# zhiyuns/AFCM

Measured on AMD Instinct MI355X. Metric: generator fwd+bwd images/sec @256^2, higher is better.
Workload: dtype bf16; 1 GPU; AFCM --model stylegan3 generator training step (fwd + L1 loss + bwd + grad all-reduce + Adam), IXI T1->T2 shape: 256x256, 4->1 channels, full-width 58.5M-param generator, random init; global_batch=16, per_gpu_batch=16, resolution=256, parallelism=dp1, world_size=1, gradient_buckets=0, comm_dtype=fp32, homogeneous_dot=True

## Files before the change

### afcm_amd/_lib.py

```python
import ctypes as C
import os

import torch

_HERE = os.path.dirname(os.path.abspath(__file__))
LIB_PATH = os.environ.get('AFCM_HIP_LIB') or os.path.join(_HERE, 'libafcm_hip.so')

F32, F16, BF16 = 0, 1, 2
E_NOKERNEL, E_INVALID = -1, -2
SIGNS_NONE, SIGNS_WRITE, SIGNS_READ = 0, 1, 2

_DTYPES = {torch.float32: F32, torch.float16: F16, torch.bfloat16: BF16}


class FilteredLReluArgs(C.Structure):
    _fields_ = [
        ('x', C.c_void_p), ('y', C.c_void_p), ('b', C.c_void_p), ('signs', C.c_void_p),
        ('fu', C.c_void_p), ('fd', C.c_void_p),
        ('dtype', C.c_int32),
        ('n', C.c_int32), ('c', C.c_int32), ('xh', C.c_int32), ('xw', C.c_int32), ('yh', C.c_int32), ('yw', C.c_int32),
        ('fuw', C.c_int32), ('fuh', C.c_int32), ('fdw', C.c_int32), ('fdh', C.c_int32),
        ('up', C.c_int32), ('down', C.c_int32),
        ('px0', C.c_int32), ('px1', C.c_int32), ('py0', C.c_int32), ('py1', C.c_int32),
        ('sx', C.c_int32), ('sy', C.c_int32), ('sh', C.c_int32), ('swb', C.c_int32),
        ('gain', C.c_float), ('slope', C.c_float), ('clamp', C.c_float),
        ('flip_filter', C.c_int32), ('sign_mode', C.c_int32),
        ('workspace', C.c_void_p), ('sign_layout', C.c_int32), ('plane_sum_slots', C.c_int32),
        ('plane_sum', C.c_void_p), ('oscale', C.c_void_p), ('skip', C.c_void_p), ('oscale2', C.c_void_p),
        ('x_pitch', C.c_int32), ('y_pitch', C.c_int32), ('skip_pitch', C.c_int32), ('row_pitch_ok', C.c_int32),
        ('clamp_flags', C.c_void_p),
    ]


AFFINE_MAX = 16


class AffineBank(C.Structure):
    _fields_ = [
        ('layers', C.c_int32), ('n', C.c_int32), ('kw', C.c_int32), ('kg', C.c_int32),
        ('w_stride_n', C.c_int64), ('w_stride_l', C.c_int64),
        ('w', C.c_void_p), ('g', C.c_void_p),
        ('weight', C.c_void_p * AFFINE_MAX), ('bias', C.c_void_p * AFFINE_MAX),
        ('cout', C.c_int32 * AFFINE_MAX), ('w_index', C.c_int32 * AFFINE_MAX),
        ('alpha', C.c_float * AFFINE_MAX), ('beta', C.c_float * AFFINE_MAX),
    ]


MODULATION_MAX = 16


class ModulationLayer(C.Structure):
    _fields_ = [('cout', C.c_int32), ('cin', C.c_int32), ('kk', C.c_int32), ('demodulate', C.c_int32)] + [
        (k, C.c_void_p) for k in ('w', 't', 'magnitude', 'w_hat', 'wsq', 'scale', 's_eff', 'd', 'r', 'g_hat', 'g_s', 'g_d', 'dw', 'dt', 'workspace')]


PACK_MAX = 32


class PackEntry(C.Structure):
    _fields_ = [('dst_fwd', C.c_void_p), ('dst_dgrad', C.c_void_p), ('w', C.c_void_p),
                ('cout', C.c_int32), ('cin', C.c_int32), ('rows_pad_fwd', C.c_int32), ('rows_pad_dgrad', C.c_int32)]


_lib = None
ABI_VERSION = 13

_i32, _i64, _f32, _vp = C.c_int32, C.c_int64, C.c_float, C.c_void_p
SIGNATURES = {
    'afcm_abi_version': (C.c_int, []),
    'afcm_last_error': (C.c_char_p, []),
    'afcm_noop': (C.c_int, [_vp]),
    'afcm_filtered_lrelu_shapes': (C.c_int, [C.POINTER(FilteredLReluArgs)]),
    'afcm_filtered_lrelu': (C.c_int, [C.POINTER(FilteredLReluArgs), _vp]),
    'afcm_filtered_lrelu_workspace_bytes': (C.c_int64, []),
    'afcm_filtered_lrelu_prepare': (C.c_int, [C.POINTER(FilteredLReluArgs), _vp]),
    'afcm_filtered_lrelu_act': (C.c_int, [_vp, _vp, _i32, _i32, _i32, _i32, _i32, _i32, _i32, _i32, _i32, _f32, _f32, _f32, _i32, _vp]),
    'afcm_upfirdn2d': (C.c_int, [_vp, _vp, _vp, _i32, _i32, _i32, _i32, _i32, _i32, _i32, _i32, _i32, _i32, _i32, _i32, _i32,
                                 _i32, _i32, _i32, _f32, _vp]),
    'afcm_bias_act': (C.c_int, [_vp, _vp, _vp, _vp, _vp, _vp, _i32, _i64, _i64, _i32, _i32, _i32, _f32, _f32, _f32, _vp]),
    'afcm_conv2d_block_k': (C.c_int, [_i32]),
    'afcm_conv2d_block_k_ks': (C.c_int, [_i32, _i32]),
    'afcm_conv2d_pack_weights_bk': (C.c_int, [_vp, _vp, _i32, _i32, _i32, _i32, _i32, _i32, _i32, _vp]),
    'afcm_conv2d_pack_weights': (C.c_int, [_vp, _vp, _i32, _i32, _i32, _i32, _i32, _i32, _vp]),
    'afcm_conv2d_pack_weights2': (C.c_int, [_vp, _vp, _vp, _i32, _i32, _i32, _i32, _i32, _i32, _vp]),
    'afcm_conv2d': (C.c_int, [_vp, _vp, _vp, _vp, _vp, _i32, _i32, _i32, _i32, _i32, _i32, _i32, _i32, _i32, _vp]),
    'afcm_conv2d_ld': (C.c_int, [_vp, _vp, _vp, _vp, _vp, _i32, _i32, _i32, _i32, _i32, _i32, _i32, _i32, _i32, _i32, _i32, _vp]),
    'afcm_conv2d_wgrad_splits': (C.c_int, [_i32, _i32, _i32, _i32]),
    'afcm_conv2d_wgrad': (C.c_int, [_vp, _vp, _vp, _vp, _i32, _i32, _i32, _i32, _i32, _i32, _i32, _i32, _vp]),
    'afcm_conv2d_wgrad_ld': (C.c_int, [_vp, _vp, _vp, _vp, _i32, _i32, _i32, _i32, _i32, _i32, _i32, _i32, _i32, _i32, _vp]),
    'afcm_conv2d_wgrad_dots_ld': (C.c_int, [_vp, _vp, _vp, _vp, _vp, _vp, _i32, _i32, _i32, _i32, _i32, _i32, _i32, _i32, _i32, _i32, _vp]),
    'afcm_scale_planes': (C.c_int, [_vp, _vp, _vp, _i32, _i32, _i64, _i32, _vp]),
    'afcm_plane_dot': (C.c_int, [_vp, _vp, _vp, _i32, _i64, _i32, _vp]),
    'afcm_plane_dot_ld': (C.c_int, [_vp, _vp, _vp, _i32, _i64, _i32, _i32, _i32, _i32, _vp]),
    'afcm_split16': (C.c_int, [_vp, _vp, _vp, _vp, _i32, _i64, _i32, _i32, _i64, _vp]),
    'afcm_conv2d_split': (C.c_int, [_vp, _vp, _vp, _vp, _vp, _i32, _i32, _i32, _i32, _i32, _i32, _i32, _i32, _i32, C.c_uint32, _i64, _vp, _vp, _vp]),
    'afcm_amax_bits': (C.c_int, [_vp, _vp, _i64, _i32, _vp, _vp]),
    'afcm_unscale': (C.c_int, [_vp, _i64, _vp, _vp, _vp]),
    'afcm_plane_dot_parts': (C.c_int, [_vp, _vp, _i64, _i32, _vp, _i32, _i64, _i32, _vp, _vp]),
    'afcm_conv2d_pack_split': (C.c_int, [_vp, _vp, _vp, _i32, _i32, _i32, _i32, _i32, _i32, C.c_uint32, _vp]),
    'afcm_plane_dot_gated_ld': (C.c_int, [_vp, _vp, _vp, _i32, _i64, _i32, _i32, _i32, _i32, _vp, _i32, _vp, _vp, _vp, _vp, _vp]),
    'afcm_weight_norm_fwd': (C.c_int, [_vp, _vp, _vp, _vp, _i32, _i32, _i32, _vp]),
    'afcm_weight_norm_bwd': (C.c_int, [_vp, _vp, _vp, _vp, _vp, _i32, _i32, _i32, _vp]),
    'afcm_style_coefs_fwd': (C.c_int, [_vp, _vp, _vp, _vp, _vp, _vp, _i32, _i32, _i32, _i32, _vp]),
    'afcm_style_coefs_bwd': (C.c_int, [_vp, _vp, _vp, _vp, _vp, _vp, _vp, _vp, _vp, _vp, _i32, _i32, _i32, _i32, _vp]),
    'afcm_layer_bwd_coefs': (C.c_int, [_vp, _vp, _vp, _vp, _i32, _vp, _vp, _vp, _vp, _vp, _i32, _i32, _vp]),
    'afcm_affine_bank_workspace_bytes': (C.c_int64, [C.POINTER(AffineBank)]),
    'afcm_affine_bank_fwd': (C.c_int, [C.POINTER(AffineBank), C.POINTER(C.c_void_p), _vp]),
    'afcm_modulation_bank_workspace_floats': (C.c_int64, [_i32, _i32, _i32, _i32]),
    'afcm_modulation_bank_fwd': (C.c_int, [C.POINTER(ModulationLayer), _i32, _i32, _vp]),
    'afcm_modulation_bank_bwd': (C.c_int, [C.POINTER(ModulationLayer), _i32, _i32, _vp]),
    'afcm_conv2d_stride2': (C.c_int, [_vp, _vp, _vp, _i32, _i32, _i32, _i32, _i32, _i32, _i32, _i32, _vp]),
    'afcm_conv2d_pack_bank': (C.c_int, [C.POINTER(PackEntry), _i32, _i32, _i32, _vp]),
    'afcm_affine_bank_bwd': (C.c_int, [C.POINTER(AffineBank), C.POINTER(C.c_void_p), C.POINTER(C.c_void_p), C.POINTER(C.c_void_p), _vp, _vp, _vp, _vp]),
    'afcm_pool_blocks_fwd': (C.c_int, [_vp, _vp, _i32, _i64, _i32, _i32, _vp]),
    'afcm_pool_blocks_bwd': (C.c_int, [_vp, _vp, _i32, _i64, _i32, _i32, _vp]),
    'afcm_l1_partials': (C.c_int, [_vp, _vp, _vp, _i64, _i32, _f32, _vp]),
    'afcm_l1_grad': (C.c_int, [_vp, _vp, _vp, _vp, _i64, _f32, _vp]),
    'afcm_axpy_planes': (C.c_int, [_vp, _vp, _vp, _vp, _i32, _i64, _i32, _vp]),
    'afcm_fc_act_fwd': (C.c_int, [_vp, _vp, _vp, _vp, _i32, _i32, _i32, _f32, _f32, _i32, _vp]),
    'afcm_fc_act_bwd': (C.c_int, [_vp, _vp, _vp, _vp, _vp, _vp, _vp, _i32, _i32, _i32, _f32, _f32, _i32, _vp]),
    'afcm_mapping_input_fwd': (C.c_int, [_vp, _vp, _vp, _vp, _vp, _i32, _i32, _i32, _i32, _f32, _f32, _vp]),
    'afcm_mapping_input_bwd_workspace_bytes': (C.c_int64, [_i32, _i32]),
    'afcm_mapping_input_bwd': (C.c_int, [_vp, _vp, _vp, _vp, _vp, _vp, _i32, _i32, _i32, _i32, _f32, _f32, _vp, _vp]),
    'afcm_adam_chunk_elems': (C.c_int32, []),
    'afcm_adam_multi': (C.c_int, [_vp, _i32, _i64, _f32, _f32, _f32, _f32, _f32, _f32, _f32, _f32, _i32, _f32, _f32, _i32, _vp]),
    'afcm_adam_multi_capturable': (C.c_int, [_vp, _i32, _i64, _vp, _f32, _f32, _f32, _f32, _f32, _i32, _f32, _f32, _i32, _vp]),
}


def load():
    global _lib
    if _lib is None:
        if not os.path.exists(LIB_PATH):
            raise RuntimeError(
                f'{LIB_PATH} is missing: the HIP kernels are not built.  Run `python -c "import __graft_entry__ as g; g.build()"` '
                f'or `make -C afcm_amd/csrc`.  afcm_amd has no CPU fallback.')
        lib = C.CDLL(LIB_PATH)
        for name, (res, args) in SIGNATURES.items():
            fn = getattr(lib, name)
            fn.restype = res
            fn.argtypes = args
        if lib.afcm_abi_version() != ABI_VERSION:
            raise RuntimeError(f'libafcm_hip.so ABI version {lib.afcm_abi_version()} does not match this package ({ABI_VERSION}); rebuild it')
        _lib = lib
    return _lib


def dtype_code(t):
    try:
        return _DTYPES[t.dtype]
    except KeyError:
        raise RuntimeError(f'afcm_amd kernels support float32/float16/bfloat16, got {t.dtype}') from None


def require_gpu(*tensors):
    for t in tensors:
        if t is not None and t.device.type != 'cuda':
            raise RuntimeError(
                f'afcm_amd ops need ROCm device tensors (got a tensor on {t.device}); there is no CPU path in this package '
                f'-- the aten reference lives in oracle/ and is test-only')


def stream_ptr(t):
    return torch.cuda.current_stream(t.device).cuda_stream


def ptr(t):
    return None if t is None else t.data_ptr()


def check(rc, what):
    if rc == 0 or rc == E_NOKERNEL:
        return rc
    if rc == E_INVALID:
        raise RuntimeError(f'{what}: {load().afcm_last_error().decode()}')
    raise RuntimeError(f'{what}: HIP error {rc - 1000} at kernel launch')


def launched(rc, what):
    if check(rc, what) == E_NOKERNEL:
        raise RuntimeError(f'{what}: no kernel for this shape (the Python gate and the C entry point disagree)')
    return rc
```

### afcm_amd/csrc/conv2d.hip

```cpp
#include <stdlib.h>
#include <string.h>

#include <type_traits>

#include "common.h"

namespace afcm {

typedef __attribute__((ext_vector_type(16))) float f32x16;
typedef __attribute__((ext_vector_type(8))) __bf16 bf16x8;
typedef __attribute__((ext_vector_type(8))) _Float16 f16x8;
typedef __attribute__((ext_vector_type(2))) float cf32x2;
typedef __attribute__((ext_vector_type(2))) __bf16 cbf16x2;
typedef __attribute__((ext_vector_type(2))) _Float16 cf16x2;

template <typename T>
__device__ __forceinline__ unsigned pack2(float lo, float hi) {
    if constexpr (std::is_same<T, bf16_t>::value) {
        union { cbf16x2 v; unsigned u; } r;
        r.v = __builtin_convertvector((cf32x2){lo, hi}, cbf16x2);
        return r.u;
    } else {
        union { cf16x2 v; unsigned u; } r;
        r.v = __builtin_convertvector((cf32x2){lo, hi}, cf16x2);
        return r.u;
    }
}

template <typename T> struct ConvCfg;
template <> struct ConvCfg<bf16_t> { static constexpr int BK = 16, PITCH = 24; };
template <> struct ConvCfg<f16_t>  { static constexpr int BK = 16, PITCH = 24; };
template <> struct ConvCfg<float>  { static constexpr int BK = 8,  PITCH = 9;  };

static inline int conv_bk(int dtype, int ks);
int conv2d_direct_small_cin(const void* x, void* y, const void* wp, const float* oscale, const float* obias, int dtype, int n, int cin, int cout,
                            int h, int w, int pad, int rows_pad, int bk, int ldx, int ldy, hipStream_t st);

constexpr int kPatchMax = 416;
constexpr int kPlaneX16 = 416;
constexpr int kPatchMaxX16 = kPlaneX16 - 4;
constexpr int kPatchMaxS2 = 704;
constexpr int kSlots = 256;

struct ConvParams {
    const void* x;
    void* y;
    const void* wp;
    const float* oscale;
    const float* obias;
    int N, Cin, Cout, H, W, P, Q;
    int ldx, ldy;
    int pad;
    int TH, TW, PWL, tilesX, tilesY;
    int Opad, nkc;
    int total_blocks;
    int o_base;
    unsigned magicTW;
    unsigned magicTX, magicTY, magicN, magicPC;
    int nkc_real; unsigned magicNK, term_parts; int part_bytes, last_part_bytes;
    const unsigned* bound_a; const unsigned* bound_b;
};
__device__ __forceinline__ float pow2_factor(unsigned bound_bits, float* inverse = nullptr) {
    const float b = __uint_as_float(bound_bits);
    int e = 15;
    if (b <= 3.4028234664e38f) frexpf(fmaxf(b, 1e-30f), &e);
    if (inverse) *inverse = ldexpf(1.f, e - 15);
    return ldexpf(1.f, 15 - e);
}

__host__ __device__ inline unsigned magic_u32(unsigned d) { return (unsigned)((0x100000000ull + d - 1) / d); }
__device__ __forceinline__ unsigned udiv_magic(unsigned n, unsigned magic) { return magic ? __umulhi(n, magic) : n; }

template <typename T, int BM_O, int KS>
__global__ __launch_bounds__(256, (sizeof(T) == 4 ? 1 : 2)) void conv2d_fwd_kernel(ConvParams p) {
    typedef ConvCfg<T> C;
    constexpr int BK = C::BK, PITCH = C::PITCH, MI = BM_O / 64, KK = KS * KS;
    constexpr bool F32 = sizeof(T) == 4;
    constexpr int EPV = 16 / sizeof(T);
    constexpr int PPR = BK / EPV;
    constexpr int NPIECES = KK * BM_O * PPR;
    constexpr int NWP = cdiv(NPIECES, 256);
    __shared__ __attribute__((aligned(16))) T lds[(KK * BM_O + kPatchMax) * PITCH];
    T* lds_w = lds;
    T* lds_p = lds + KK * BM_O * PITCH;

    const int tid = threadIdx.x, lane = tid & 63, wave = tid >> 6;
    const int wo = wave & 1, wpx = wave >> 1;
    const int r32 = lane & 31, h = lane >> 5;

    int bid = blockIdx.x;
    const int tx = __builtin_amdgcn_readfirstlane(bid % p.tilesX); bid /= p.tilesX;
    const int ty = __builtin_amdgcn_readfirstlane(bid % p.tilesY); bid /= p.tilesY;
    const int n = __builtin_amdgcn_readfirstlane(bid % p.N);
    const int ob = __builtin_amdgcn_readfirstlane(bid / p.N);
    const int y0 = ty * p.TH, x0 = tx * p.TW;
    const int o0 = ob * BM_O;
    const int PH = p.TH + KS - 1, PWL = p.PWL;
    const int xorg = (x0 - p.pad) & ~1;
    const int xoff = (x0 - p.pad) - xorg;

    int bbase[4], pyv[4], pxv[4];
#pragma unroll
    for (int ti = 0; ti < 4; ti++) {
        const int j = wpx * 128 + ti * 32 + r32;
        int py = j / p.TW, px = j - py * p.TW;
        const bool valid = j < p.TH * p.TW;
        if (!valid) { py = 0; px = 0; }
        pyv[ti] = valid ? y0 + py : p.P;
        pxv[ti] = x0 + px;
        bbase[ti] = (py * PWL + px + xoff) * PITCH + h * (F32 ? 1 : 8);
    }
    int abase[MI];
#pragma unroll
    for (int mi = 0; mi < MI; mi++) abase[mi] = (wo * (BM_O / 2) + mi * 32 + r32) * PITCH + h * (F32 ? 1 : 8);

    f32x16 acc[MI][4];
#pragma unroll
    for (int mi = 0; mi < MI; mi++)
#pragma unroll
        for (int ti = 0; ti < 4; ti++)
#pragma unroll
            for (int e = 0; e < 16; e++) acc[mi][ti][e] = 0.f;

    constexpr int PPT = BM_O * PPR;
    constexpr int TPI = 256 / PPT;
    const int wq = tid % PPT, wtap0 = tid / PPT;
    const int wsrc0 = ((wtap0 * p.Opad) + o0 + wq / PPR) * BK + (wq % PPR) * EPV;
    const int wdst0 = (wtap0 * BM_O + wq / PPR) * PITCH + (wq % PPR) * EPV;
    const int wsrc_step = TPI * p.Opad * BK, wdst_step = TPI * BM_O * PITCH;
    const size_t wchunk = (size_t)KK * p.Opad * BK;
    const int cg = F32 ? 0 : (tid >> 5) & 1, pg = F32 ? tid : (tid & 31) + 32 * (tid >> 6);
    const int pcols = PWL >> 2;
    const int prow = pg / pcols, pcol4 = pg - prow * pcols;
    const bool pvalid = prow < PH;
    const int iy = y0 - p.pad + prow, ix = xorg + 4 * pcol4;
    const bool rowok = pvalid && (unsigned)iy < (unsigned)p.H;
    const T* xn = (const T*)p.x + (size_t)n * p.Cin * p.H * p.W;
    const long long pix_off = (long long)(rowok ? iy : 0) * p.W + ix;
    const int pdst = (prow * PWL + 4 * pcol4) * PITCH + cg * 8;

    unsigned wreg[NWP][4];
    unsigned preg[8][F32 ? 4 : 2];
    constexpr unsigned kOob = 0x80000000u;
    const bool d0ok = rowok && (unsigned)ix < (unsigned)p.W, d1ok = rowok && (unsigned)(ix + 2) < (unsigned)p.W;
    const unsigned pmask0 = d0ok ? ~0u : 0u, pmask1 = d1ok ? ~0u : 0u;
    const bool any_partial = __builtin_amdgcn_ballot_w64(d0ok != d1ok) != 0;
    const bool lshift = !d0ok && d1ok;
    const bool any_lshift = __builtin_amdgcn_ballot_w64(lshift) != 0;
    const unsigned pvoff = (d0ok || d1ok) ? (unsigned)(((long long)cg * 8 * p.H * p.W + pix_off + (lshift ? 2 : 0)) * (long long)sizeof(T)) : kOob;
    const long long img_bytes = (long long)p.Cin * p.H * p.W * (long long)sizeof(T);
    const __amdgpu_buffer_rsrc_t xrs = __builtin_amdgcn_make_buffer_rsrc((void*)xn, 0, (int)(img_bytes > 0x7fffffffll ? 0x7fffffffll : img_bytes), 0x00020000);
    const int hw2 = p.H * p.W * (int)sizeof(T);

    auto issue_loads = [&](int kc) __attribute__((always_inline)) {
        const T* wsrcp = (const T*)p.wp + (size_t)kc * wchunk;
#pragma unroll
        for (int i = 0; i < NWP; i++)
            if ((NPIECES % 256 == 0) || tid + i * 256 < NPIECES) {
                const uint4 t = *(const uint4*)(wsrcp + wsrc0 + i * wsrc_step);
                wreg[i][0] = t.x; wreg[i][1] = t.y; wreg[i][2] = t.z; wreg[i][3] = t.w;
            }
        if constexpr (F32) {
#pragma unroll
            for (int c = 0; c < 8; c++) {
                const int ch = kc * BK + cg * 8 + c;
                const bool chok = rowok && ch < p.Cin;
                const T* src = xn + ((long long)ch * p.H * p.W + pix_off);
#pragma unroll
                for (int e = 0; e < 4; e++) preg[c][e] = (chok && (unsigned)(ix + e) < (unsigned)p.W) ? *(const unsigned*)(src + e) : 0u;
            }
        } else {
            const bool tailchunk = (kc + 1) * BK > p.Cin;
#pragma unroll
            for (int c = 0; c < 8; c++) {
                typedef __attribute__((ext_vector_type(2))) unsigned u32x2;
                const u32x2 v = __builtin_amdgcn_raw_buffer_load_b64(xrs, pvoff, (kc * BK + c) * hw2, 0);
                preg[c][0] = v.x; preg[c][1] = v.y;
            }
            if (tailchunk) {
#pragma unroll
                for (int c = 0; c < 8; c++)
                    if (kc * BK + cg * 8 + c >= p.Cin) { preg[c][0] = 0u; preg[c][1] = 0u; }
            }
        }
    };
    auto write_lds = [&]() __attribute__((always_inline)) {
#pragma unroll
        for (int i = 0; i < NWP; i++)
            if ((NPIECES % 256 == 0) || tid + i * 256 < NPIECES) {
                if (F32) {
                    unsigned* d = (unsigned*)(lds_w + wdst0 + i * wdst_step);
                    d[0] = wreg[i][0]; d[1] = wreg[i][1]; d[2] = wreg[i][2]; d[3] = wreg[i][3];
                } else {
                    *(uint4*)(lds_w + wdst0 + i * wdst_step) = make_uint4(wreg[i][0], wreg[i][1], wreg[i][2], wreg[i][3]);
                }
            }
        if (pvalid) {
            if (F32) {
#pragma unroll
                for (int e = 0; e < 4; e++) {
                    unsigned* d = (unsigned*)(lds_p + pdst + e * PITCH);
#pragma unroll
                    for (int c = 0; c < 8; c++) d[c] = preg[c][e];
                }
            } else {
                if (any_lshift) {
#pragma unroll
                    for (int c = 0; c < 8; c++) preg[c][1] = lshift ? preg[c][0] : preg[c][1];
                }
                if (any_partial) {
#pragma unroll
                    for (int c = 0; c < 8; c++) { preg[c][0] &= pmask0; preg[c][1] &= pmask1; }
                }
#pragma unroll
                for (int e = 0; e < 4; e++) {
                    const unsigned sel = (e & 1) ? 0x07060302u : 0x05040100u;
                    uint4 v;
                    v.x = __builtin_amdgcn_perm(preg[1][e >> 1], preg[0][e >> 1], sel);
                    v.y = __builtin_amdgcn_perm(preg[3][e >> 1], preg[2][e >> 1], sel);
                    v.z = __builtin_amdgcn_perm(preg[5][e >> 1], preg[4][e >> 1], sel);
                    v.w = __builtin_amdgcn_perm(preg[7][e >> 1], preg[6][e >> 1], sel);
                    *(uint4*)(lds_p + pdst + e * PITCH) = v;
                }
            }
        }
    };

    issue_loads(0);
    write_lds();
    __syncthreads();
    for (int kc = 0; kc < p.nkc; kc++) {
        if (kc + 1 < p.nkc) issue_loads(kc + 1);
#pragma unroll
        for (int r = 0; r < KS; r++)
#pragma unroll
            for (int s = 0; s < KS; s++) {
                const int tap = r * KS + s;
                const int tapoff = (r * PWL + s) * PITCH;
                if constexpr (F32) {
#pragma unroll
                    for (int k2 = 0; k2 < BK / 2; k2++) {
                        float a[MI], b[4];
#pragma unroll
                        for (int mi = 0; mi < MI; mi++) a[mi] = lds_w[tap * BM_O * PITCH + abase[mi] + 2 * k2];
#pragma unroll
                        for (int ti = 0; ti < 4; ti++) b[ti] = lds_p[bbase[ti] + tapoff + 2 * k2];
#pragma unroll
                        for (int mi = 0; mi < MI; mi++)
#pragma unroll
                            for (int ti = 0; ti < 4; ti++)
                                acc[mi][ti] = __builtin_amdgcn_mfma_f32_32x32x2f32(a[mi], b[ti], acc[mi][ti], 0, 0, 0);
                    }
                } else {
                    typedef typename std::conditional<std::is_same<T, bf16_t>::value, bf16x8, f16x8>::type frag_t;
                    frag_t a[MI], b[4];
#pragma unroll
                    for (int mi = 0; mi < MI; mi++) a[mi] = *(const frag_t*)(lds_w + tap * BM_O * PITCH + abase[mi]);
#pragma unroll
                    for (int ti = 0; ti < 4; ti++) b[ti] = *(const frag_t*)(lds_p + bbase[ti] + tapoff);
#pragma unroll
                    for (int mi = 0; mi < MI; mi++)
#pragma unroll
                        for (int ti = 0; ti < 4; ti++) {
                            if constexpr (std::is_same<T, bf16_t>::value)
                                acc[mi][ti] = __builtin_amdgcn_mfma_f32_32x32x16_bf16(a[mi], b[ti], acc[mi][ti], 0, 0, 0);
                            else
                                acc[mi][ti] = __builtin_amdgcn_mfma_f32_32x32x16_f16(a[mi], b[ti], acc[mi][ti], 0, 0, 0);
                        }
                }
            }
        __syncthreads();
        if (kc + 1 < p.nkc) {
            write_lds();
            __syncthreads();
        }
    }

    T* yn = (T*)p.y + (size_t)n * p.Cout * p.P * p.Q;
    int poff[4];
#pragma unroll
    for (int ti = 0; ti < 4; ti++) poff[ti] = (pyv[ti] < p.P && pxv[ti] < p.Q) ? pyv[ti] * p.Q + pxv[ti] : -1;
    const float* osn = p.oscale ? p.oscale + (size_t)n * p.Cout : nullptr;
    const int pq = p.P * p.Q;
#pragma unroll
    for (int mi = 0; mi < MI; mi++) {
        float sc[16], ob[16];
        const int obase = o0 + wo * (BM_O / 2) + mi * 32 + 4 * h;
#pragma unroll
        for (int reg = 0; reg < 16; reg++) { sc[reg] = 1.f; ob[reg] = 0.f; }
        if (osn != nullptr) {
#pragma unroll
            for (int reg = 0; reg < 16; reg++) sc[reg] = osn[min(obase + (reg & 3) + 8 * (reg >> 2), p.Cout - 1)];
        }
        if (p.obias != nullptr) {
#pragma unroll
            for (int reg = 0; reg < 16; reg++) ob[reg] = p.obias[min(obase + (reg & 3) + 8 * (reg >> 2), p.Cout - 1)];
        }
#pragma unroll
        for (int reg = 0; reg < 16; reg++) {
            const int o = obase + (reg & 3) + 8 * (reg >> 2);
            if (o < p.Cout) {
                T* yo = yn + (size_t)o * pq;
#pragma unroll
                for (int ti = 0; ti < 4; ti++)
                    if (poff[ti] >= 0) yo[poff[ti]] = from_f32<T>(acc[mi][ti][reg] * sc[reg] + ob[reg]);
            }
        }
    }
}

template <typename T, int BM_O, bool SPLIT = false, bool FASTEPI = false>
__global__ __launch_bounds__(256, 2) void conv2d_fwd16x_kernel(ConvParams p) {
    static_assert(sizeof(T) == 2, "16-bit types only");
    static_assert(!(SPLIT && FASTEPI), "the fp32-output epilogue has no fast form");
    typedef typename std::conditional<SPLIT, float, T>::type TO;
    constexpr int KS = 3, KK = 9, BK = 32, MO = BM_O / 32, NT = 8, BRING = MO == 4 ? 4 : 3;
    constexpr int ARING = MO == 2 ? 6 : 9;
    static_assert((KK * MO) % ARING == 0 && ARING >= 2 * MO, "static slots; a tap's fragments and the next tap's are live together");
    constexpr int PLANE_B = kPlaneX16 * 16;
    constexpr int BUF_B = 4 * PLANE_B;
    static_assert(PLANE_B % 256 == 0 && kPatchMaxX16 % 4 == 0, "planes: a multiple of 256 bytes apart, patch + sink inside");
    typedef typename std::conditional<std::is_same<T, bf16_t>::value, bf16x8, f16x8>::type frag_t;
    typedef __attribute__((ext_vector_type(4))) float f32x4;
    typedef __attribute__((ext_vector_type(4))) unsigned u32x4;
    typedef __attribute__((ext_vector_type(2))) unsigned u32x2;
    __shared__ __attribute__((aligned(256))) unsigned char lds[2 * BUF_B];

    const int tid = threadIdx.x, lane = tid & 63;
    const int wave = __builtin_amdgcn_readfirstlane(tid >> 6);
    const int wo = wave & 1, wpx = wave >> 1;
    const int c16 = lane & 15, g = lane >> 4;
    const int PH = p.TH + KS - 1, PWL = p.PWL;

    constexpr bool PERSIST = BM_O == 64 || BM_O == 96;
    struct Tile { int y0, x0, n, o0; };
    auto decode = [&](int it) __attribute__((always_inline)) -> Tile {
        const int bid = xcd_order(it, p.total_blocks);
        const unsigned q0 = udiv_magic((unsigned)bid, p.magicTX);
        const int tx = __builtin_amdgcn_readfirstlane(bid - (int)q0 * p.tilesX);
        const unsigned q1 = udiv_magic(q0, p.magicTY);
        const int ty = __builtin_amdgcn_readfirstlane((int)q0 - (int)q1 * p.tilesY);
        const unsigned q2 = udiv_magic(q1, p.magicN);
        const int n = __builtin_amdgcn_readfirstlane((int)q1 - (int)q2 * p.N);
        const int ob = __builtin_amdgcn_readfirstlane((int)q2);
        return Tile{ty * p.TH, tx * p.TW, n, p.o_base + ob * BM_O};
    };

    f32x4 acc[MO][NT];

    const int wtap_b = p.Opad * BK * 2;
    const __amdgpu_buffer_rsrc_t wrs = __builtin_amdgcn_make_buffer_rsrc((void*)p.wp, 0, p.nkc * KK * wtap_b, 0x00020000);
    const unsigned wlane = (unsigned)(((wo * (BM_O / 2) + c16) * BK + g * 8) * 2);
    auto load_a = [&](int o0s, int kc, int tap, int mo) __attribute__((always_inline)) {
        return __builtin_bit_cast(frag_t, __builtin_amdgcn_raw_buffer_load_b128(wrs, wlane, (kc * KK + tap) * wtap_b + (o0s + mo * 16) * (BK * 2), 0));
    };

    const int cg = (tid >> 5) & 1, pg = (tid & 31) + 32 * (tid >> 6);
    const int pcols = PWL >> 2;
    constexpr unsigned kOob = 0x80000000u;
    const long long img_bytes = (long long)p.Cin * p.H * p.ldx * 2ll + (SPLIT ? (long long)p.last_part_bytes : 0ll);
    const int img_records = (int)(img_bytes > 0x7fffffffll ? 0x7fffffffll : img_bytes);
    const int hw2 = p.H * p.ldx * 2;
    const int rot = (pg >> 1) & 1;
    const int pgd = 4 * pg < kPatchMaxX16 ? 4 * pg : kPatchMaxX16;
    const unsigned pdst_a = (unsigned)(pgd * 16 + cg * PLANE_B + rot * 16);
    const unsigned sel_a = rot ? 0x07060302u : 0x05040100u;
    unsigned pvoff = kOob, pm_lo = 0, pm_hi = 0;
    bool lshift = false;
    __amdgpu_buffer_rsrc_t xrs = wrs;
    auto stage_tile = [&](const Tile& t) __attribute__((always_inline)) {
        int tid_o = tid;
        asm volatile("" : "+v"(tid_o));
        const int pg_o = (tid_o & 31) + 32 * (tid_o >> 6), cg_o = (tid_o >> 5) & 1;
        const int prow = (int)udiv_magic((unsigned)pg_o, p.magicPC), pcol4 = pg_o - prow * pcols;
        const bool pvalid = prow < PH;
        const int cg = cg_o;
        const int xorg = (t.x0 - p.pad) & ~1;
        const int iy = t.y0 - p.pad + prow, ix = xorg + 4 * pcol4;
        const bool rowok = pvalid && (unsigned)iy < (unsigned)p.H;
        const long long pix_off = (long long)(rowok ? iy : 0) * p.ldx + ix;
        const bool d0ok = rowok && (unsigned)ix < (unsigned)p.W, d1ok = rowok && (unsigned)(ix + 2) < (unsigned)p.W;
        lshift = !d0ok && d1ok;
        pm_lo = (d0ok && !lshift) ? ~0u : 0u;
        pm_hi = d1ok ? ~0u : 0u;
        pvoff = (d0ok || d1ok) ? (unsigned)(((long long)cg * 8 * p.H * p.ldx + pix_off + (lshift ? 2 : 0)) * 2ll) : kOob;
        xrs = __builtin_amdgcn_make_buffer_rsrc((void*)((const T*)p.x + (size_t)t.n * p.Cin * p.H * p.ldx), 0, img_records, 0x00020000);
    };

    auto issue_patch = [&](unsigned (&pr)[8][2], int kc, bool live, int item) __attribute__((always_inline)) {
        int kcr = kc, sbase = 0;
        if constexpr (SPLIT) {
            const int term = (int)udiv_magic((unsigned)kc, p.magicNK);
            kcr = kc - term * p.nkc_real;
            sbase = (int)((p.term_parts >> (4 * term)) & 15u) * p.part_bytes;
        }
        const int cbase = kcr * BK + item * 16 + cg * 8;
        const int climit = live ? p.Cin : 0;
        const unsigned voff = live ? pvoff : kOob;
#pragma unroll
        for (int c = 0; c < 8; c++) {
            unsigned off = voff;
            if constexpr (SPLIT) off = (cbase + c < climit) ? pvoff : kOob;
            const u32x2 v = __builtin_amdgcn_raw_buffer_load_b64(xrs, off, sbase + (kcr * BK + item * 16 + c) * hw2, 0);
            pr[c][0] = v.x; pr[c][1] = v.y;
        }
    };
    auto mask_ch = [&](unsigned (&pr)[8][2], int c) __attribute__((always_inline)) {
        const unsigned lo = pr[c][0] & pm_lo;
        const unsigned hi = (lshift ? pr[c][0] : pr[c][1]) & pm_hi;
        pr[c][0] = lo; pr[c][1] = hi;
    };
    auto write_px = [&](unsigned (&pr)[8][2], int e, int sbyte) __attribute__((always_inline)) {
        const unsigned sel = (e & 1) ? (sel_a ^ 0x02020202u) : sel_a;
        u32x4 v;
        v.x = __builtin_amdgcn_perm(pr[1][e >> 1], pr[0][e >> 1], sel);
        v.y = __builtin_amdgcn_perm(pr[3][e >> 1], pr[2][e >> 1], sel);
        v.z = __builtin_amdgcn_perm(pr[5][e >> 1], pr[4][e >> 1], sel);
        v.w = __builtin_amdgcn_perm(pr[7][e >> 1], pr[6][e >> 1], sel);
        *(u32x4*)(lds + ((e & 1) ? (pdst_a ^ 16u) : pdst_a) + (unsigned)sbyte + (e >> 1) * 32) = v;
    };
    unsigned bbyte[NT];
    auto set_bbyte = [&](const Tile& t, int buf) __attribute__((always_inline)) {
        const int xoff = (t.x0 - p.pad) & 1;
        int lane_o = tid;
        asm volatile("" : "+v"(lane_o));
        lane_o &= 63;
        if constexpr (FASTEPI) {
            const unsigned lanepart = (unsigned)((lane_o & 15) * 16 + (lane_o >> 4) * PLANE_B);
#pragma unroll
            for (int ti = 0; ti < NT; ti++) {
                const int b16 = wpx * 128 + ti * 16;
                int py = (int)__umulhi((unsigned)b16, p.magicTW), px = b16 - py * p.TW;
                if (b16 >= p.TH * p.TW) { py = 0; px = 0; }
                bbyte[ti] = lanepart + (unsigned)((py * PWL + px + xoff) * 16 + buf * BUF_B);
            }
            return;
        }
#pragma unroll
        for (int ti = 0; ti < NT; ti++) {
            const int j = wpx * 128 + ti * 16 + (lane_o & 15);
            int py = (int)__umulhi((unsigned)j, p.magicTW), px = j - py * p.TW;
            if (j >= p.TH * p.TW) { py = 0; px = 0; }
            bbyte[ti] = (unsigned)((py * PWL + px + xoff) * 16 + (lane_o >> 4) * PLANE_B + buf * BUF_B);
        }
    };

    int item = blockIdx.x;
    Tile S = decode(item);
    stage_tile(S);
    frag_t ar[ARING];
    unsigned preg[8][2];
    {
        unsigned preg1[8][2];
        issue_patch(preg, 0, true, 0);
        issue_patch(preg1, 0, true, 1);
#pragma unroll
        for (int q = 0; q < ARING; q++) ar[q] = load_a(S.o0, 0, q / MO, q % MO);
#pragma unroll
        for (int c = 0; c < 8; c++) { mask_ch(preg, c); mask_ch(preg1, c); }
#pragma unroll
        for (int e = 0; e < 4; e++) { write_px(preg, e, 0); write_px(preg1, e, 2 * PLANE_B); }
    }
    int cb = 0;
    set_bbyte(S, cb);
    __syncthreads();

    const int last = p.nkc - 1;
    const unsigned rowstep = (unsigned)(PWL * 16);
    for (;;) {
        const int item_n = item + (int)gridDim.x;
        const bool has_next = PERSIST && item_n < p.total_blocks;
#pragma unroll
        for (int mo = 0; mo < MO; mo++)
#pragma unroll
            for (int ti = 0; ti < NT; ti++) acc[mo][ti] = (f32x4){0.f, 0.f, 0.f, 0.f};
        for (int kc = 0; kc < p.nkc; kc++) {
            const bool fin = kc == last;
            int o0_n = S.o0;
            if (PERSIST && fin) {
                const Tile N = decode(has_next ? item_n : item);
                stage_tile(N);
                o0_n = N.o0;
            }
            const int nxt_b = (cb ^ 1) * BUF_B;
            const bool more = !fin || has_next;
            const int knext = fin ? 0 : kc + 1;
            const unsigned bufstep = (unsigned)((cb ? -BUF_B : BUF_B) - 2 * (int)rowstep);
            frag_t b[BRING];
#pragma unroll
            for (int s = 0; s < BRING; s++) b[s] = *(const frag_t*)(lds + bbyte[s]);
            __builtin_amdgcn_sched_barrier(0);
#pragma unroll
            for (int tap = 0; tap < KK; tap++) {
#pragma unroll
                for (int ti = 0; ti < NT; ti++) {
                    const int s = tap * NT + ti;
#pragma unroll
                    for (int mo = 0; mo < MO; mo++) {
                        if constexpr (std::is_same<T, bf16_t>::value)
                            acc[mo][ti] = __builtin_amdgcn_mfma_f32_16x16x32_bf16(ar[(tap * MO + mo) % ARING], b[s % BRING], acc[mo][ti], 0, 0, 0);
                        else
                            acc[mo][ti] = __builtin_amdgcn_mfma_f32_16x16x32_f16(ar[(tap * MO + mo) % ARING], b[s % BRING], acc[mo][ti], 0, 0, 0);
                    }
                    const int s2 = s + BRING;
                    if (s2 < KK * NT) {
                        const int t2 = s2 / NT, ti2 = s2 % NT;
                        if (t2 > 0 && t2 % KS == 0) bbyte[ti2] += rowstep;
                        b[s % BRING] = *(const frag_t*)(lds + bbyte[ti2] + (t2 % KS) * 16);
                    }
                    if (tap == 0 && ti == 0) issue_patch(preg, knext, more, 0);
                    if (tap == 5 && ti == 0) issue_patch(preg, knext, more, 1);
                    if (tap == 4 || tap == 8) {
                        if (ti < 4) { mask_ch(preg, 2 * ti); mask_ch(preg, 2 * ti + 1); }
                        else write_px(preg, ti - 4, nxt_b + (tap == 8 ? 2 * PLANE_B : 0));
                    }
                    if (tap == 8 && ti >= 4) { bbyte[2 * (ti - 4)] += bufstep; bbyte[2 * (ti - 4) + 1] += bufstep; }
                    if (ti == NT - 1) {
#pragma unroll
                        for (int mo = 0; mo < MO; mo++) {
                            const int q = tap * MO + mo, q2 = q + ARING;
                            ar[q % ARING] = (q2 < KK * MO) ? load_a(S.o0, kc, q2 / MO, q2 % MO) : load_a(o0_n, knext, (q2 - KK * MO) / MO, q2 % MO);
                        }
                    }
                    __builtin_amdgcn_sched_barrier(0);
                }
            }
            cb ^= 1;
            __syncthreads();
        }
        int lane_e = tid;
        asm volatile("" : "+v"(lane_e));
        lane_e &= 63;
        const int c16e = lane_e & 15, ge = lane_e >> 4;
        const int y0 = S.y0, x0 = S.x0, n = S.n, o0 = S.o0;
        if constexpr (!SPLIT) {
            typedef __attribute__((ext_vector_type(4))) short s16x4;
            typedef __attribute__((ext_vector_type(4))) unsigned eu32x4;
            constexpr int EROW = 64;
            unsigned char* const ebuf = lds + (cb ^ 1) * BUF_B + wave * (64 * EROW);
            const int pq = p.P * p.ldy;
            const __amdgpu_buffer_rsrc_t yrs = __builtin_amdgcn_make_buffer_rsrc((void*)((T*)p.y + (size_t)n * p.Cout * pq), 0, p.Cout * pq * 2, 0x00020000);
            const __amdgpu_buffer_rsrc_t srs = __builtin_amdgcn_make_buffer_rsrc((void*)(p.oscale ? p.oscale + (size_t)n * p.Cout : (const float*)p.y), 0, p.oscale ? p.Cout * 4 : 0, 0x00020000);
            const __amdgpu_buffer_rsrc_t brs = __builtin_amdgcn_make_buffer_rsrc((void*)(p.obias ? p.obias : (const float*)p.y), 0, p.obias ? p.Cout * 4 : 0, 0x00020000);
            constexpr unsigned kGOut = 0x80000000u, kOOut = 0xc0000000u;
            const bool has_sc = p.oscale != nullptr, has_ob = p.obias != nullptr;
            f32x4 sc[MO], ob[MO];
#pragma unroll
            for (int mo = 0; mo < MO; mo++) {
                const unsigned sboff = (unsigned)((o0 + wo * (BM_O / 2) + mo * 16 + 4 * ge) * 4);
                sc[mo] = (f32x4){1.f, 1.f, 1.f, 1.f};
                ob[mo] = (f32x4){0.f, 0.f, 0.f, 0.f};
                if (has_sc) sc[mo] = __builtin_bit_cast(f32x4, __builtin_amdgcn_raw_buffer_load_b128(srs, sboff, 0, 0));
                if (has_ob) ob[mo] = __builtin_bit_cast(f32x4, __builtin_amdgcn_raw_buffer_load_b128(brs, sboff, 0, 0));
            }
            const int i16 = lane_e & 15, chalf = (lane_e >> 4) & 1, hh = lane_e >> 5;
            const int q4 = i16 >> 2, p4 = i16 & 3;
            unsigned rd_off[2];
#pragma unroll
            for (int r = 0; r < 2; r++) {
                const int prw = 8 * hh + 4 * r + q4;
                rd_off[r] = prw * EROW + (((chalf * 4 + p4) ^ ((prw >> 1) & 7)) << 3);
            }
            unsigned wr_off[2];
#pragma unroll
            for (int k = 0; k < 2; k++) wr_off[k] = (unsigned)(c16e * EROW + (((4 * k + ge) ^ ((c16e >> 1) & 7)) << 3));
            unsigned gbyte[8], gfullm = 0, slow_any = 0;
#pragma unroll
            for (int it = 0; it < (FASTEPI ? 0 : 8); it++) {
                const int j0 = wpx * 128 + (2 * it + hh) * 8;
                const int gpy = (int)__umulhi((unsigned)j0, p.magicTW), gpx = j0 - gpy * p.TW;
                const int gy = y0 + gpy, gx = x0 + gpx;
                const bool in_tile = j0 < p.TH * p.TW && gy < p.P;
                const bool valid = in_tile && gx < p.Q;
                const bool straddle = gpx + 8 > p.TW;
                const bool slow = in_tile && (straddle || (valid && gx + 8 > p.ldy));
                gbyte[it] = valid ? (unsigned)((gy * p.ldy + gx) * 2) : kGOut;
                if (!slow) gfullm |= 1u << it;
                if (__builtin_amdgcn_ballot_w64(slow) != 0) slow_any |= 1u << it;
            }
#pragma unroll
            for (int mi = 0; mi < (MO + 1) / 2; mi++) {
                const int rowbase = o0 + wo * (BM_O / 2) + mi * 32;
                const int o = rowbase + chalf * 16 + i16;
                const unsigned obyte = (o < p.Cout && mi * 32 + chalf * 16 < BM_O / 2) ? (unsigned)(o * pq * 2) : kOOut;
#pragma unroll
                for (int half = 0; half < 2; half++) {
#pragma unroll
                    for (int k = 0; k < 2; k++) {
                        const int mo = 2 * mi + k;
                        if (mo >= MO) continue;
#pragma unroll
                        for (int t4 = 0; t4 < 4; t4++) {
                            const int ti = 4 * half + t4;
                            uint2 w;
                            w.x = pack2<T>(acc[mo][ti][0] * sc[mo][0] + ob[mo][0], acc[mo][ti][1] * sc[mo][1] + ob[mo][1]);
                            w.y = pack2<T>(acc[mo][ti][2] * sc[mo][2] + ob[mo][2], acc[mo][ti][3] * sc[mo][3] + ob[mo][3]);
                            *(uint2*)(ebuf + wr_off[k] + t4 * (16 * EROW)) = w;
                        }
                    }
#pragma unroll
                    for (int i4 = 0; i4 < 4; i4++) {
                        const int it = 4 * half + i4;
                        union { s16x4 v[2]; eu32x4 q; } u;
#pragma unroll
                        for (int r = 0; r < 2; r++)
                            u.v[r] = __builtin_amdgcn_ds_read_tr16_b64_v4i16((__attribute__((address_space(3))) s16x4*)(ebuf + i4 * (16 * EROW) + rd_off[r]));
                        if constexpr (FASTEPI) {
                            const int b16 = wpx * 128 + 16 * it;
                            const int gpy = (int)__umulhi((unsigned)b16, p.magicTW), gpxs = b16 - gpy * p.TW;
                            const int gy = y0 + gpy, gxs = x0 + gpxs;
                            if (b16 < p.TH * p.TW && gy < p.P && gxs < p.Q) {
                                unsigned vo = obyte + 16u * (unsigned)hh;
                                if (gxs + 8 >= p.Q && hh) vo = kGOut;
                                __builtin_amdgcn_raw_buffer_store_b128(u.q, yrs, vo, (gy * p.ldy + gxs) * 2, 0);
                            }
                            continue;
                        }
                        const bool full = (gfullm >> it) & 1;
                        __builtin_amdgcn_raw_buffer_store_b128(u.q, yrs, full ? obyte + gbyte[it] : kGOut, 0, 0);
                        if ((slow_any >> it) & 1) {
                            if (!full) {
#pragma unroll
                                for (int w2 = 0; w2 < 4; w2++) {
                                    const int j = wpx * 128 + (2 * it + hh) * 8 + 2 * w2;
                                    const int py = (int)__umulhi((unsigned)j, p.magicTW), px = j - py * p.TW;
                                    const bool ok = j < p.TH * p.TW && y0 + py < p.P && x0 + px < p.Q;
                                    __builtin_amdgcn_raw_buffer_store_b32(u.q[w2], yrs, ok ? obyte + (unsigned)(((y0 + py) * p.ldy + x0 + px) * 2) : kGOut, 0, 0);
                                }
                            }
                        }
                    }
                }
            }
        } else {
            TO* yn = (TO*)p.y + (size_t)n * p.Cout * p.P * p.ldy;
            int poff[NT];
#pragma unroll
            for (int ti = 0; ti < NT; ti++) {
                const int j = wpx * 128 + ti * 16 + c16e;
                const int py = (int)__umulhi((unsigned)j, p.magicTW), px = j - py * p.TW;
                poff[ti] = (j < p.TH * p.TW && y0 + py < p.P && x0 + px < p.Q) ? (y0 + py) * p.ldy + x0 + px : -1;
            }
            const float* osn = p.oscale ? p.oscale + (size_t)n * p.Cout : nullptr;
            const int pq = p.P * p.ldy;
            float ia = 1.f, ib = 1.f;
            if (p.bound_a) pow2_factor(p.bound_a[0], &ia);
            if (p.bound_b) pow2_factor(p.bound_b[0], &ib);
            const float inv = ia * ib;
#pragma unroll
            for (int mo = 0; mo < MO; mo++) {
                float sc[4], ob[4];
                const int obase = o0 + wo * (BM_O / 2) + mo * 16 + 4 * ge;
#pragma unroll
                for (int reg = 0; reg < 4; reg++) {
                    sc[reg] = (osn != nullptr ? osn[min(obase + reg, p.Cout - 1)] : 1.f) * inv;
                    ob[reg] = p.obias != nullptr ? p.obias[min(obase + reg, p.Cout - 1)] : 0.f;
                }
#pragma unroll
                for (int reg = 0; reg < 4; reg++) {
                    const int o = obase + reg;
                    if (o < p.Cout) {
                        TO* yo = yn + (size_t)o * pq;
#pragma unroll
                        for (int ti = 0; ti < NT; ti++)
                            if (poff[ti] >= 0) yo[poff[ti]] = from_f32<TO>(acc[mo][ti][reg] * sc[reg] + ob[reg]);
                    }
                }
            }
        }
        if (!has_next) break;
        if (!SPLIT) __syncthreads();
        S = decode(item_n);
        item = item_n;
        set_bbyte(S, cb);
    }
}

template <typename T, int BM_O>
__global__ __launch_bounds__(256, 2) void conv2d_fwd16s2_kernel(ConvParams p) {
    static_assert(sizeof(T) == 2, "16-bit types only");
    typedef ConvCfg<T> C;
    constexpr int KS = 3, KK = 9, BK = C::BK, PITCH = C::PITCH, MI = BM_O / 64, RING = 3;
    constexpr int NT = 2, PXW = 32 * NT, STRIDE = 2, NITEM = 2, PMAX = kPatchMaxS2;
    typedef typename std::conditional<std::is_same<T, bf16_t>::value, bf16x8, f16x8>::type frag_t;
    typedef __attribute__((ext_vector_type(2))) unsigned u32x2;
    __shared__ __attribute__((aligned(16))) T lds[2 * PMAX * PITCH + 4 * PITCH];

    const int tid = threadIdx.x, lane = tid & 63;
    const int wave = __builtin_amdgcn_readfirstlane(tid >> 6);
    const int wo = wave & 1, wpx = wave >> 1;
    const int r32 = lane & 31, h = lane >> 5;

    int bid = blockIdx.x;
    {
        const int total = gridDim.x;
        bid = xcd_order(bid, total);
    }
    const int tx = __builtin_amdgcn_readfirstlane(bid % p.tilesX); bid /= p.tilesX;
    const int ty = __builtin_amdgcn_readfirstlane(bid % p.tilesY); bid /= p.tilesY;
    const int n = __builtin_amdgcn_readfirstlane(bid % p.N);
    const int ob = __builtin_amdgcn_readfirstlane(bid / p.N);
    const int y0 = ty * p.TH, x0 = tx * p.TW;
    const int o0 = ob * BM_O;
    const int PH = (p.TH - 1) * STRIDE + KS, PWL = p.PWL;
    const int xorg = (x0 * STRIDE - p.pad) & ~1;
    const int xoff = (x0 * STRIDE - p.pad) - xorg;

    int bbase[NT], pyv[NT], pxv[NT];
#pragma unroll
    for (int ti = 0; ti < NT; ti++) {
        const int j = wpx * PXW + ti * 32 + r32;
        int py = j / p.TW, px = j - py * p.TW;
        const bool valid = j < p.TH * p.TW;
        if (!valid) { py = 0; px = 0; }
        pyv[ti] = valid ? y0 + py : p.P;
        pxv[ti] = x0 + px;
        bbase[ti] = (py * STRIDE * PWL + px * STRIDE + xoff) * PITCH + h * 8;
    }

    f32x16 acc[MI][NT];
#pragma unroll
    for (int mi = 0; mi < MI; mi++)
#pragma unroll
        for (int ti = 0; ti < NT; ti++)
#pragma unroll
            for (int e = 0; e < 16; e++) acc[mi][ti][e] = 0.f;

    const T* wlane = (const T*)p.wp + (size_t)(o0 + wo * (BM_O / 2) + r32) * BK + h * 8;
    const size_t wtap = (size_t)p.Opad * BK;
    auto load_a = [&](int kc, int tap, int mi) __attribute__((always_inline)) {
        return *(const frag_t*)(wlane + ((size_t)kc * KK + tap) * wtap + mi * 32 * BK);
    };

    const int cg = (tid >> 5) & 1, pg = (tid & 31) + 32 * (tid >> 6);
    const int pcols = PWL >> 2;
    const T* xn = (const T*)p.x + (size_t)n * p.Cin * p.H * p.ldx;
    constexpr unsigned kOob = 0x80000000u;
    const long long img_bytes = (long long)p.Cin * p.H * p.ldx * 2ll;
    const __amdgpu_buffer_rsrc_t xrs = __builtin_amdgcn_make_buffer_rsrc((void*)xn, 0, (int)(img_bytes > 0x7fffffffll ? 0x7fffffffll : img_bytes), 0x00020000);
    const int hw2 = p.H * p.ldx * 2;
    bool pvalid[NITEM], lshift[NITEM];
    int pdst[NITEM];
    unsigned pmask0[NITEM], pmask1[NITEM], pvoff[NITEM];
#pragma unroll
    for (int it = 0; it < NITEM; it++) {
        const int item = pg + 128 * it;
        const int prow = item / pcols, pcol4 = item - prow * pcols;
        pvalid[it] = prow < PH;
        const int iy = y0 * STRIDE - p.pad + prow, ix = xorg + 4 * pcol4;
        const bool rowok = pvalid[it] && (unsigned)iy < (unsigned)p.H;
        const long long pix_off = (long long)(rowok ? iy : 0) * p.ldx + ix;
        pdst[it] = (prow * PWL + 4 * pcol4) * PITCH + cg * 8;
        const bool d0ok = rowok && (unsigned)ix < (unsigned)p.W, d1ok = rowok && (unsigned)(ix + 2) < (unsigned)p.W;
        pmask0[it] = d0ok ? ~0u : 0u; pmask1[it] = d1ok ? ~0u : 0u;
        lshift[it] = !d0ok && d1ok;
        pvoff[it] = (d0ok || d1ok) ? (unsigned)(((long long)cg * 8 * p.H * p.ldx + pix_off + (lshift[it] ? 2 : 0)) * 2ll) : kOob;
    }

    unsigned preg[NITEM][8][2];
    auto issue_patch = [&](int kc, bool live) __attribute__((always_inline)) {
        const int cbase = kc * BK + cg * 8;
        const int climit = live ? p.Cin : 0;
#pragma unroll
        for (int it = 0; it < NITEM; it++)
#pragma unroll
            for (int c = 0; c < 8; c++) {
                const unsigned off = (cbase + c < climit) ? pvoff[it] : kOob;
                const u32x2 v = __builtin_amdgcn_raw_buffer_load_b64(xrs, off, (kc * BK + c) * hw2, 0);
                preg[it][c][0] = v.x; preg[it][c][1] = v.y;
            }
    };
    auto write_patch = [&](int kc, T* dstbuf, int bufbase) __attribute__((always_inline)) {
#pragma unroll
        for (int it = 0; it < NITEM; it++) {
#pragma unroll
            for (int c = 0; c < 8; c++) {
                const unsigned lo = lshift[it] ? 0u : (preg[it][c][0] & pmask0[it]);
                const unsigned hi = (lshift[it] ? preg[it][c][0] : preg[it][c][1]) & pmask1[it];
                preg[it][c][0] = lo; preg[it][c][1] = hi;
            }
#pragma unroll
            for (int e = 0; e < 4; e++) {
                const unsigned sel = (e & 1) ? 0x07060302u : 0x05040100u;
                uint4 v;
                v.x = __builtin_amdgcn_perm(preg[it][1][e >> 1], preg[it][0][e >> 1], sel);
                v.y = __builtin_amdgcn_perm(preg[it][3][e >> 1], preg[it][2][e >> 1], sel);
                v.z = __builtin_amdgcn_perm(preg[it][5][e >> 1], preg[it][4][e >> 1], sel);
                v.w = __builtin_amdgcn_perm(preg[it][7][e >> 1], preg[it][6][e >> 1], sel);
                *(uint4*)(lds + (pvalid[it] ? bufbase + pdst[it] + e * PITCH : 2 * PMAX * PITCH)) = v;
            }
        }
    };

    frag_t ar[RING][MI];
    issue_patch(0, true);
#pragma unroll
    for (int t = 0; t < RING; t++)
#pragma unroll
        for (int mi = 0; mi < MI; mi++) ar[t][mi] = load_a(0, t, mi);
    write_patch(0, lds, 0);
    __syncthreads();

    const int last = p.nkc - 1;
    for (int kc = 0; kc < p.nkc; kc++) {
        const T* cur = lds + (kc & 1) * (PMAX * PITCH);
        T* nxt = lds + ((kc + 1) & 1) * (PMAX * PITCH);
        const bool more = kc < last;
        frag_t b[NT];
#pragma unroll
        for (int ti = 0; ti < NT; ti++) b[ti] = *(const frag_t*)(cur + bbase[ti]);
        issue_patch(kc + (int)more, more);
        __builtin_amdgcn_sched_group_barrier(0x100, NT, 0);
        __builtin_amdgcn_sched_group_barrier(0x020, 8 * NITEM, 0);
#pragma unroll
        for (int tap = 0; tap < KK; tap++) {
            const int nr = (tap + 1) / KS, ns = (tap + 1) - nr * KS;
            const int tapoff_n = (nr * PWL + ns) * PITCH;
            frag_t a[MI];
#pragma unroll
            for (int mi = 0; mi < MI; mi++) a[mi] = ar[tap % RING][mi];
            {
                const int nt = (tap + RING) % KK;
                const int nk = (tap + RING < KK) ? kc : (more ? kc + 1 : kc);
#pragma unroll
                for (int mi = 0; mi < MI; mi++) ar[tap % RING][mi] = load_a(nk, nt, mi);
            }
#pragma unroll
            for (int ti = 0; ti < NT; ti++) {
#pragma unroll
                for (int mi = 0; mi < MI; mi++) {
                    if constexpr (std::is_same<T, bf16_t>::value)
                        acc[mi][ti] = __builtin_amdgcn_mfma_f32_32x32x16_bf16(a[mi], b[ti], acc[mi][ti], 0, 0, 0);
                    else
                        acc[mi][ti] = __builtin_amdgcn_mfma_f32_32x32x16_f16(a[mi], b[ti], acc[mi][ti], 0, 0, 0);
                }
                if (tap + 1 < KK) b[ti] = *(const frag_t*)(cur + bbase[ti] + tapoff_n);
            }
            if (tap == 5) {
                write_patch(kc + 1, nxt, ((kc + 1) & 1) * (PMAX * PITCH));
                __builtin_amdgcn_sched_group_barrier(0x020, MI, 0);
#pragma unroll
                for (int ti = 0; ti < NT; ti++) {
#pragma unroll
                    for (int mi = 0; mi < MI; mi++) {
                        __builtin_amdgcn_sched_group_barrier(0x008, 1, 0);
                        __builtin_amdgcn_sched_group_barrier(0x002, 20, 0);
                    }
                    __builtin_amdgcn_sched_group_barrier(0x100, 1, 0);
                }
                __builtin_amdgcn_sched_group_barrier(0x200, 4 * NITEM, 0);
            } else {
                __builtin_amdgcn_sched_group_barrier(0x020, MI, 0);
#pragma unroll
                for (int ti = 0; ti < NT; ti++) {
                    __builtin_amdgcn_sched_group_barrier(0x008, MI, 0);
                    if (tap + 1 < KK) __builtin_amdgcn_sched_group_barrier(0x100, 1, 0);
                }
            }
        }
        __syncthreads();
    }

    if ((p.TW & 7) == 0 && (p.Q & 1) == 0) {
        typedef __attribute__((ext_vector_type(4))) short s16x4;
        constexpr int EROW = 64;
        unsigned char* ebuf = (unsigned char*)lds + wave * (PXW * EROW);
        T* yn = (T*)p.y + (size_t)n * p.Cout * p.P * p.ldy;
        const float* osn = p.oscale ? p.oscale + (size_t)n * p.Cout : nullptr;
        const int pq = p.P * p.ldy;
        const int i16 = lane & 15, chalf = (lane >> 4) & 1, hh = lane >> 5;
        const int q4 = i16 >> 2, p4 = i16 & 3;
        unsigned rd_off[2];
#pragma unroll
        for (int r = 0; r < 2; r++) {
            const int prow = 8 * hh + 4 * r + q4;
            rd_off[r] = prow * EROW + (((chalf * 4 + p4) ^ ((prow >> 1) & 7)) << 3);
        }
        int goff[2 * NT];
        unsigned gfullm = 0;
        int gxv[2 * NT];
#pragma unroll
        for (int it = 0; it < 2 * NT; it++) {
            const int j0 = wpx * PXW + (2 * it + hh) * 8;
            const int gpy = (int)__umulhi((unsigned)j0, p.magicTW), gpx = j0 - gpy * p.TW;
            const int gy = y0 + gpy, gx = x0 + gpx;
            goff[it] = (j0 < p.TH * p.TW && gy < p.P && gx < p.Q) ? gy * p.ldy + gx : -1;
            gxv[it] = gx;
            if (gx + 8 <= p.ldy) gfullm |= 1u << it;
        }
        const int wr_pix = r32;
#pragma unroll
        for (int mi = 0; mi < MI; mi++) {
            float sc[16], ob[16];
            const int obase = o0 + wo * (BM_O / 2) + mi * 32 + 4 * h;
#pragma unroll
            for (int reg = 0; reg < 16; reg++) { sc[reg] = 1.f; ob[reg] = 0.f; }
            if (osn != nullptr) {
#pragma unroll
                for (int reg = 0; reg < 16; reg++) sc[reg] = osn[min(obase + (reg & 3) + 8 * (reg >> 2), p.Cout - 1)];
            }
            if (p.obias != nullptr) {
#pragma unroll
                for (int reg = 0; reg < 16; reg++) ob[reg] = p.obias[min(obase + (reg & 3) + 8 * (reg >> 2), p.Cout - 1)];
            }
#pragma unroll
            for (int ti = 0; ti < NT; ti++) {
                const int pix = ti * 32 + wr_pix;
                const int sw = (pix >> 1) & 7;
#pragma unroll
                for (int k4 = 0; k4 < 4; k4++) {
                    uint2 w;
                    w.x = pack2<T>(acc[mi][ti][4 * k4 + 0] * sc[4 * k4 + 0] + ob[4 * k4 + 0], acc[mi][ti][4 * k4 + 1] * sc[4 * k4 + 1] + ob[4 * k4 + 1]);
                    w.y = pack2<T>(acc[mi][ti][4 * k4 + 2] * sc[4 * k4 + 2] + ob[4 * k4 + 2], acc[mi][ti][4 * k4 + 3] * sc[4 * k4 + 3] + ob[4 * k4 + 3]);
                    *(uint2*)(ebuf + pix * EROW + (((h + 2 * k4) ^ sw) << 3)) = w;
                }
            }
            const int o = o0 + wo * (BM_O / 2) + mi * 32 + chalf * 16 + i16;
            T* const yo = yn + (size_t)min(o, p.Cout - 1) * pq;
#pragma unroll
            for (int it = 0; it < 2 * NT; it++) {
                union { s16x4 v[2]; uint4 q; } u;
#pragma unroll
                for (int r = 0; r < 2; r++)
                    u.v[r] = __builtin_amdgcn_ds_read_tr16_b64_v4i16((__attribute__((address_space(3))) s16x4*)(ebuf + it * (16 * EROW) + rd_off[r]));
                if (goff[it] >= 0 && o < p.Cout) {
                    T* dst = yo + goff[it];
                    if ((gfullm >> it) & 1) {
                        *(uint4*)dst = u.q;
                    } else {
                        const unsigned vv[4] = {u.q.x, u.q.y, u.q.z, u.q.w};
#pragma unroll
                        for (int w2 = 0; w2 < 4; w2++)
                            if (gxv[it] + 2 * w2 < p.Q) ((unsigned*)dst)[w2] = vv[w2];
                    }
                }
            }
        }
        return;
    }
    T* yn = (T*)p.y + (size_t)n * p.Cout * p.P * p.ldy;
    int poff[NT];
#pragma unroll
// ... 1317 lines not shown
                });
            } else {
                frag_t a[2][R];
#pragma unroll
                for (int ob2 = 0; ob2 < 2; ob2++)
#pragma unroll
                    for (int rr = 0; rr < R; rr++) a[ob2][rr] = *(const frag_t*)(buf + a_off[ob2] + rr * (64 * ROWB));
                uint4 lo_n = *(const uint4*)(buf + x0_off[0]);
                uint4 hi_n = *(const uint4*)(buf + x1_off[0][0]);
                static_for<0, 2 * XR>([&](auto itc) __attribute__((always_inline)) {
                    constexpr int it = decltype(itc)::value, xr = it >> 1, ib2 = it & 1, NIT = 2 * XR;
                    const uint4 lo = lo_n, hi = hi_n;
                    if constexpr (it + 1 < NIT) {
                        constexpr int xr1 = (it + 1) >> 1, ib1 = (it + 1) & 1;
                        lo_n = *(const uint4*)(buf + x0_off[ib1] + xr1 * (64 * ROWB));
                        hi_n = *(const uint4*)(buf + x1_off[ib1][xr1]);
                    }
                    __builtin_amdgcn_sched_barrier(0);
                    if constexpr (LATE) {
                        static_assert(!LATE || NPIECE == NIT - 1, "one piece per iteration after the first");
                        if constexpr (it > 0) issue_piece(std::integral_constant<int, it - 1>{});
                    } else
                        issue_range(std::integral_constant<int, (it * NPIECE) / NIT>{}, std::integral_constant<int, ((it + 1) * NPIECE) / NIT>{});
                    asm volatile("" : : "v"(lo.x), "v"(lo.y), "v"(lo.z));
                    const unsigned d[5] = {lo.w, hi.x, hi.y, hi.z, hi.w};
#pragma unroll
                    for (int sft = 0; sft < KS; sft++) {
                        union { unsigned u[4]; frag_t f; } bw;
#pragma unroll
                        for (int w = 0; w < 4; w++)
                            bw.u[w] = (sft == 0) ? d[w] : (sft == 1) ? __builtin_amdgcn_alignbyte(d[w + 1], d[w], 2) : d[w + 1];
#pragma unroll
                        for (int rr = 0; rr < R; rr++) {
                            const int r = xr - rr;
                            if (r >= 0 && r < KS) {
#pragma unroll
                                for (int ob2 = 0; ob2 < 2; ob2++) mma(a[ob2][rr], bw.f, r * KS + sft, 2 * ob2 + ib2);
                            }
                        }
                    }
                    if constexpr (LATE && it == 0) begin_loads(step + NBUF - 1 < s1);
                    __builtin_amdgcn_sched_barrier(0);
                });
            }
        } else if constexpr (!TAIL) {
            static_for<0, 2>([&](auto kqc) __attribute__((always_inline)) {
                constexpr int kq = decltype(kqc)::value;
                if ((kq * 2 + th) * 16 >= vq) {
                    issue_range(std::integral_constant<int, (kq * XR * NPIECE) / (2 * XR)>{}, std::integral_constant<int, ((kq + 1) * XR * NPIECE) / (2 * XR)>{});
                    return;
                }
                frag_t a[R];
#pragma unroll
                for (int rr = 0; rr < R; rr++) a[rr] = *(const frag_t*)(buf + a_off[kq] + rr * (64 * ROWB));
                static_for<0, XR>([&](auto xrc) __attribute__((always_inline)) {
                    constexpr int xr = decltype(xrc)::value;
                    constexpr int it = kq * XR + xr, NIT = 2 * XR;
                    issue_range(std::integral_constant<int, (it * NPIECE) / NIT>{}, std::integral_constant<int, ((it + 1) * NPIECE) / NIT>{});
                    const frag_t b = *(const frag_t*)(buf + x0_off[kq] + xr * (64 * ROWB));
                    constexpr int rr = xr;
                    if constexpr (std::is_same<T, bf16_t>::value) acc[0] = __builtin_amdgcn_mfma_f32_32x32x16_bf16(a[rr], b, acc[0], 0, 0, 0);
                    else acc[0] = __builtin_amdgcn_mfma_f32_32x32x16_f16(a[rr], b, acc[0], 0, 0, 0);
                });
            });
        } else {
            frag_t a[2][R];
#pragma unroll
            for (int rr = 0; rr < R; rr++) a[0][rr] = *(const frag_t*)(buf + a_off[0] + rr * (64 * ROWB));
            uint4 lo_n = *(const uint4*)(buf + x0_off[0]);
            uint4 hi_n = *(const uint4*)(buf + x1_off[0][0]);
            static_for<0, 2>([&](auto kqc) __attribute__((always_inline)) {
                constexpr int kq = decltype(kqc)::value;
                if ((kq * 2 + th) * 16 >= vq) {
                    issue_range(std::integral_constant<int, (kq * XR * NPIECE) / (2 * XR)>{}, std::integral_constant<int, ((kq + 1) * XR * NPIECE) / (2 * XR)>{});
                    if constexpr (kq == 0) {
#pragma unroll
                        for (int rr = 0; rr < R; rr++) a[1][rr] = *(const frag_t*)(buf + a_off[1] + rr * (64 * ROWB));
                        lo_n = *(const uint4*)(buf + x0_off[1]);
                        hi_n = *(const uint4*)(buf + x1_off[1][0]);
                    }
                    return;
                }
                static_for<0, XR>([&](auto xrc) __attribute__((always_inline)) {
                    constexpr int xr = decltype(xrc)::value;
                    const uint4 lo = lo_n, hi = hi_n;
                    if constexpr (xr + 1 < XR) {
                        lo_n = *(const uint4*)(buf + x0_off[kq] + (xr + 1) * (64 * ROWB));
                        hi_n = *(const uint4*)(buf + x1_off[kq][xr + 1 < XR ? xr + 1 : xr]);
                    } else if constexpr (kq == 0) {
                        lo_n = *(const uint4*)(buf + x0_off[1]);
                        hi_n = *(const uint4*)(buf + x1_off[1][0]);
                    }
                    if constexpr (kq == 0 && xr == 1) {
#pragma unroll
                        for (int rr = 0; rr < R; rr++) a[1][rr] = *(const frag_t*)(buf + a_off[1] + rr * (64 * ROWB));
                    }
                    __builtin_amdgcn_sched_barrier(0);
                    row_mfmas(kqc, xrc, lo, hi, a[kq]);
                    __builtin_amdgcn_sched_barrier(0);
                });
            });
        }
        if (NBUF == 3) asm volatile("s_waitcnt vmcnt(%0)" : : "n"(NPIECE));
        else { asm volatile("s_waitcnt vmcnt(0)"); f_q0 = c_q0; f_live = c_live; f_bufa = c_bufa; }
        fix_edge();
        __syncthreads();
        if (++cbuf == NBUF) cbuf = 0;
    }
    asm volatile("s_waitcnt vmcnt(0)");
    __syncthreads();
    {
        float* red = (float*)lds;
        constexpr int TPR_CAP = (NBUF * BUF) / (4 * 16 * 64 * (int)sizeof(float));
        constexpr int TPR = TPR_CAP < KK ? TPR_CAP : KK;
        static_assert(TPR >= 1, "LDS too small for the half-sum");
        const int wv4 = wo + 2 * wi;
#pragma unroll
        for (int t0 = 0; t0 < KK; t0 += TPR) {
            if (t0 > 0) __syncthreads();
            if (th == 1) {
#pragma unroll
                for (int t = t0; t < t0 + TPR && t < KK; t++)
#pragma unroll
                    for (int reg = 0; reg < 16; reg++) red[((wv4 * TPR + (t - t0)) * 16 + reg) * 64 + lane] = acc[t][reg];
            }
            __syncthreads();
            if (th == 0) {
#pragma unroll
                for (int t = t0; t < t0 + TPR && t < KK; t++)
#pragma unroll
                    for (int reg = 0; reg < 16; reg++) acc[t][reg] += red[((wv4 * TPR + (t - t0)) * 16 + reg) * 64 + lane];
            }
        }
    }
    if (th == 0) {
        float* out = p.part + (size_t)split * p.O * p.I * KK;
#pragma unroll
        for (int reg = 0; reg < 16; reg++) {
            const int o = o0 + wo * 32 + (X16 ? 16 * (reg >> 3) + 4 * g4 + (reg & 3) : (reg & 3) + 8 * (reg >> 2) + 4 * h);
            const int i = i0 + wi * 32 + (X16 ? 16 * ((reg >> 2) & 1) + c16 : r32);
            if (o < p.O && i < p.I) {
                float* dst = out + ((size_t)o * p.I + i) * KK;
#pragma unroll
                for (int t = 0; t < KK; t++) dst[t] = acc[t][reg];
            }
        }
    }
}

struct WgradSlabs { int I, KK, fo, fi, splits, splits_p; };
__device__ __forceinline__ int slabs_of(const WgradSlabs& w, long long idx) {
    if (w.splits_p == w.splits) return w.splits;
    const int oi = (int)(idx / w.KK), o = oi / w.I, i = oi - o * w.I;
    return ((o >> 6) < w.fo && (i >> 6) < w.fi) ? w.splits : w.splits_p;
}
__global__ __launch_bounds__(256) void wgrad_reduce_kernel(float* __restrict__ dw, const float* __restrict__ part, long long numel, WgradSlabs w) {
    for (long long idx = (long long)blockIdx.x * blockDim.x + threadIdx.x; idx < numel; idx += (long long)gridDim.x * blockDim.x) {
        float s = 0.f;
        const int splits = slabs_of(w, idx);
        for (int k = 0; k < splits; k++) s += part[(size_t)k * numel + idx];
        dw[idx] = s;
    }
}

template <int COLS>
__global__ __launch_bounds__(256) void wgrad_reduce4_kernel(float* __restrict__ dw, const float* __restrict__ part, long long numel4, WgradSlabs w) {
    constexpr int GROUPS = 256 / COLS;
    typedef __attribute__((ext_vector_type(4))) float f32x4v;
    __shared__ f32x4v red[GROUPS][COLS];
    const int col = threadIdx.x % COLS, grp = threadIdx.x / COLS;
    const long long c4 = (long long)blockIdx.x * COLS + col;
    f32x4v s0 = {0.f, 0.f, 0.f, 0.f}, s1 = s0;
    if (c4 < numel4) {
        const f32x4v* src = (const f32x4v*)part + c4;
        int ne[4];
#pragma unroll
        for (int e = 0; e < 4; e++) ne[e] = slabs_of(w, 4 * c4 + e);
        const int splits = min(min(ne[0], ne[1]), min(ne[2], ne[3]));
        const int most = max(max(ne[0], ne[1]), max(ne[2], ne[3]));
        for (int k2 = splits + grp; k2 < most; k2 += GROUPS) {
            const f32x4v v = src[(size_t)k2 * numel4];
#pragma unroll
            for (int e = 0; e < 4; e++) s1[e] += k2 < ne[e] ? v[e] : 0.f;
        }
        int k = grp;
        for (; k + 3 * GROUPS < splits; k += 4 * GROUPS) {
            const f32x4v v0 = src[(size_t)k * numel4], v1 = src[(size_t)(k + GROUPS) * numel4];
            const f32x4v v2 = src[(size_t)(k + 2 * GROUPS) * numel4], v3 = src[(size_t)(k + 3 * GROUPS) * numel4];
            s0 += v0; s1 += v1; s0 += v2; s1 += v3;
        }
        for (; k < splits; k += GROUPS) s0 += src[(size_t)k * numel4];
    }
    s0 += s1;
    if (GROUPS > 1) {
        red[grp][col] = s0;
        __syncthreads();
        if (grp == 0 && c4 < numel4) {
#pragma unroll
            for (int g = 1; g < GROUPS; g++) s0 += red[g][col];
            ((f32x4v*)dw)[c4] = s0;
        }
    } else if (c4 < numel4) {
        ((f32x4v*)dw)[c4] = s0;
    }
}


template <typename T, int KK>
__global__ __launch_bounds__(1024) void wgrad_reduce_dots_kernel(float* __restrict__ dw, float* __restrict__ dots, const float* __restrict__ part,
                                                                 const float* __restrict__ w, int N, int O, int I, int splits_img) {
    constexpr int NW = 16;
    __shared__ float red[NW - 1][64][KK];
    const int i = blockIdx.x, lane = threadIdx.x & 63, q = threadIdx.x >> 6;
    const size_t slab = (size_t)O * I * KK;
    float dotp[4];
#pragma unroll
    for (int k = 0; k < 4; k++) dotp[k] = 0.f;
    for (int ob = 0; ob < O; ob += 64) {
        const int o = ob + lane;
        const bool live = o < O;
        const size_t e0 = ((size_t)(live ? o : O - 1) * I + i) * KK;
        float wq[KK], tot[KK];
#pragma unroll
        for (int t = 0; t < KK; t++) { wq[t] = live ? to_f32(from_f32<T>(w[e0 + t])) : 0.f; tot[t] = 0.f; }
#pragma unroll
        for (int k = 0; k < 4; k++) {
            const int n = q + NW * k;
            if (n >= N) break;
            float acc[KK];
#pragma unroll
            for (int t = 0; t < KK; t++) acc[t] = 0.f;
            for (int sp = 0; sp < splits_img; sp++) {
                const float* src = part + (size_t)(n * splits_img + sp) * slab + e0;
#pragma unroll
                for (int t = 0; t < KK; t++) acc[t] += src[t];
            }
            float d = 0.f;
#pragma unroll
            for (int t = 0; t < KK; t++) { tot[t] += acc[t]; d = fmaf(wq[t], acc[t], d); }
            dotp[k] += d;
        }
        if (ob > 0) __syncthreads();
        if (q > 0) {
#pragma unroll
            for (int t = 0; t < KK; t++) red[q - 1][lane][t] = tot[t];
        }
        __syncthreads();
        if (q == 0 && live) {
#pragma unroll
            for (int t = 0; t < KK; t++) {
                float s = tot[t];
#pragma unroll
                for (int k = 0; k < NW - 1; k++) s += red[k][lane][t];
                dw[e0 + t] = s;
            }
        }
    }
#pragma unroll
    for (int k = 0; k < 4; k++) {
        const int n = q + NW * k;
        if (n >= N) break;
        float d = dotp[k];
#pragma unroll
        for (int off = 32; off > 0; off >>= 1) d += __shfl_xor(d, off);
        if (lane == 0) dots[(size_t)n * I + i] = d;
    }
}

static void choose_tile(int P, int Q, int KS, int* TH, int* TW, int* PWL, int patch_max = kPatchMax) {
    double best = -1;
    constexpr double gran_bonus = 0.03;
    for (int tw = 2; tw <= 128; tw += 2) {
        int th = kSlots / tw;
        if (th > P) th = P;
        for (; th >= 1; th--) {
            const int pwl = round_up(tw + KS, 4);
            if ((th + KS - 1) * pwl > patch_max) continue;
            const double tiles = (double)cdiv(P, th) * cdiv(Q, tw);
            const double util = (double)P * Q / (tiles * kSlots);
            const double score = util + 1e-4 * tw + ((tw & 7) == 0 ? gran_bonus : 0.0);
            if (score > best) { best = score; *TH = th; *TW = tw; *PWL = pwl; }
            break;
        }
    }
}

static void choose_tile_s2(int P, int Q, int* TH, int* TW, int* PWL) {
    double best = -1;
    for (int tw = 2; tw <= 64; tw += 2) {
        int th = 128 / tw;
        if (th > P) th = P;
        for (; th >= 1; th--) {
            const int pwl = round_up((tw - 1) * 2 + 4, 4);
            if (((th - 1) * 2 + 3) * pwl > kPatchMaxS2) continue;
            const double tiles = (double)cdiv(P, th) * cdiv(Q, tw);
            const double util = (double)P * Q / (tiles * 128);
            const double score = util + 1e-4 * tw + ((tw & 7) == 0 ? 0.03 : 0.0);
            if (score > best) { best = score; *TH = th; *TW = tw; *PWL = pwl; }
            break;
        }
    }
}

static int conv_persistent_grid(long long items, int per_cu) {
    static int cus[16] = {0};
    int dev = 0;
    (void)hipGetDevice(&dev);
    int n = (dev >= 0 && dev < 16) ? cus[dev] : 0;
    if (n == 0) {
        if (hipDeviceGetAttribute(&n, hipDeviceAttributeMultiprocessorCount, dev) != hipSuccess || n <= 0) n = 256;
        if (dev >= 0 && dev < 16) cus[dev] = n;
    }
    const long long slots = (long long)round_up(n * per_cu, 8);
    return (int)(items < slots ? items : slots);
}

static bool conv_fast_epilogue(const ConvParams& p) {
    return (p.TW & 15) == 0 && (p.ldy & 7) == 0 && (p.Q & 1) == 0;
}

template <typename T, int BM_O>
static int launch_conv(ConvParams p, int ks, hipStream_t st, int o_base = 0, int row_blocks = 0) {
    const long long blocks = (long long)p.tilesX * p.tilesY * p.N * (row_blocks ? row_blocks : cdiv(p.Cout, BM_O));
    p.o_base = o_base;
    AFCM_REQUIRE(blocks > 0 && blocks < (1ll << 31), "conv2d: grid of %lld blocks is out of range", blocks);
    dim3 grid((unsigned)blocks), block(256);
    p.total_blocks = (int)blocks;
    if constexpr (sizeof(T) == 2) {
        if (ks == 3) {
            const dim3 g16 = BM_O == 64 ? dim3((unsigned)conv_persistent_grid(blocks, 3)) : grid;
            if (conv_fast_epilogue(p)) hipLaunchKernelGGL((conv2d_fwd16x_kernel<T, BM_O, false, true>), g16, block, 0, st, p);
            else hipLaunchKernelGGL((conv2d_fwd16x_kernel<T, BM_O>), g16, block, 0, st, p);
            return hip_status(hipGetLastError());
        }
    }
    if (ks == 3) hipLaunchKernelGGL((conv2d_fwd_kernel<T, BM_O, 3>), grid, block, 0, st, p);
    else hipLaunchKernelGGL((conv2d_fwd_kernel<T, BM_O, 1>), grid, block, 0, st, p);
    return hip_status(hipGetLastError());
}

}

using namespace afcm;

extern "C" int afcm_conv2d_block_k(int32_t dtype) { return dtype == AFCM_F32 ? ConvCfg<float>::BK : ConvCfg<bf16_t>::BK; }
static inline int afcm::conv_bk(int dtype, int ks) { return (dtype != AFCM_F32 && ks == 3) ? 32 : afcm_conv2d_block_k(dtype); }
extern "C" int afcm_conv2d_block_k_ks(int32_t dtype, int32_t ks) { return conv_bk(dtype, ks); }

template <typename T>
static void launch_pack8(void* dst0, void* dst1, const float* w, int cout, int cin, int ks, int rows_pad0, int rows_pad1, int BK, hipStream_t st) {
    const int omax = dst0 ? rows_pad0 : round_up(cout, BK), imax = dst1 ? rows_pad1 : round_up(cin, BK);
    constexpr int BKT = ConvCfg<T>::BK;
    const int ti = BK > 16 ? PackTile<32>::TI : PackTile<BKT>::TI, to = BK > 16 ? PackTile<32>::TO : PackTile<BKT>::TO;
    dim3 grid((unsigned)cdiv(imax > cin ? imax : cin, ti), (unsigned)cdiv(omax > cout ? omax : cout, to)), block(256);
    if constexpr (sizeof(T) == 2) {
        if (BK == 32) {
            hipLaunchKernelGGL((conv2d_pack_tile_kernel<T, 9, 32>), grid, block, 0, st, (T*)dst0, (T*)dst1, w, cout, cin, rows_pad0, rows_pad1);
            return;
        }
    }
    if (ks == 3) hipLaunchKernelGGL((conv2d_pack_tile_kernel<T, 9, BKT>), grid, block, 0, st, (T*)dst0, (T*)dst1, w, cout, cin, rows_pad0, rows_pad1);
    else hipLaunchKernelGGL((conv2d_pack_tile_kernel<T, 1, BKT>), grid, block, 0, st, (T*)dst0, (T*)dst1, w, cout, cin, rows_pad0, rows_pad1);
}

static int pack_weights2_bk(void* dst_fwd, void* dst_dgrad, const float* w, int32_t dtype, int32_t cout, int32_t cin, int32_t ks,
                            int32_t rows_pad_fwd, int32_t rows_pad_dgrad, int BK, void* stream);
extern "C" int afcm_conv2d_pack_weights2(void* dst_fwd, void* dst_dgrad, const float* w, int32_t dtype, int32_t cout, int32_t cin, int32_t ks,
                                         int32_t rows_pad_fwd, int32_t rows_pad_dgrad, void* stream) {
    return pack_weights2_bk(dst_fwd, dst_dgrad, w, dtype, cout, cin, ks, rows_pad_fwd, rows_pad_dgrad, conv_bk(dtype, ks), stream);
}
extern "C" int afcm_conv2d_pack_weights_bk(void* dst, const float* w, int32_t dtype, int32_t cout, int32_t cin, int32_t ks, int32_t mode,
                                           int32_t rows_pad, int32_t block_k, void* stream) {
    AFCM_REQUIRE(dst != nullptr && w != nullptr, "conv2d_pack_weights: null pointer");
    AFCM_REQUIRE(mode == 0 || mode == 1, "mode must be 0 (forward) or 1 (data gradient)");
    AFCM_REQUIRE(block_k == afcm_conv2d_block_k(dtype) || block_k == conv_bk(dtype, ks), "conv2d_pack_weights_bk: K-chunk %d is not one of this dtype's", block_k);
    return mode == 0 ? pack_weights2_bk(dst, nullptr, w, dtype, cout, cin, ks, rows_pad, 0, block_k, stream)
                     : pack_weights2_bk(nullptr, dst, w, dtype, cout, cin, ks, 0, rows_pad, block_k, stream);
}
static int pack_weights2_bk(void* dst_fwd, void* dst_dgrad, const float* w, int32_t dtype, int32_t cout, int32_t cin, int32_t ks,
                            int32_t rows_pad_fwd, int32_t rows_pad_dgrad, int BK, void* stream) {
    AFCM_REQUIRE(w != nullptr && (dst_fwd != nullptr || dst_dgrad != nullptr), "conv2d_pack_weights: null pointer");
    AFCM_REQUIRE(dtype == AFCM_F32 || dtype == AFCM_F16 || dtype == AFCM_BF16, "dtype must be float32, float16 or bfloat16");
    AFCM_REQUIRE(ks == 1 || ks == 3, "only 1x1 and 3x3 kernels are supported");
    AFCM_REQUIRE(cout > 0 && cin > 0, "conv2d_pack_weights: empty weights");
    AFCM_REQUIRE(dst_fwd == nullptr || (rows_pad_fwd >= cout && rows_pad_fwd % 64 == 0), "rows_pad must be a multiple of 64 covering the rows");
    AFCM_REQUIRE(dst_dgrad == nullptr || (rows_pad_dgrad >= cin && rows_pad_dgrad % 64 == 0), "rows_pad must be a multiple of 64 covering the rows");
    AFCM_REQUIRE((((uintptr_t)dst_fwd | (uintptr_t)dst_dgrad) & 31) == 0, "conv2d_pack_weights: destinations must be 32-byte aligned");
    hipStream_t st = (hipStream_t)stream;
    switch (dtype) {
        case AFCM_F32: launch_pack8<float>(dst_fwd, dst_dgrad, w, cout, cin, ks, rows_pad_fwd, rows_pad_dgrad, BK, st); break;
        case AFCM_F16: launch_pack8<f16_t>(dst_fwd, dst_dgrad, w, cout, cin, ks, rows_pad_fwd, rows_pad_dgrad, BK, st); break;
        default: launch_pack8<bf16_t>(dst_fwd, dst_dgrad, w, cout, cin, ks, rows_pad_fwd, rows_pad_dgrad, BK, st); break;
    }
    return hip_status(hipGetLastError());
}

extern "C" int afcm_conv2d_pack_weights(void* dst, const float* w, int32_t dtype, int32_t cout, int32_t cin, int32_t ks,
                                        int32_t mode, int32_t rows_pad, void* stream) {
    AFCM_REQUIRE(dst != nullptr && w != nullptr, "conv2d_pack_weights: null pointer");
    AFCM_REQUIRE(mode == 0 || mode == 1, "mode must be 0 (forward) or 1 (data gradient)");
    return mode == 0 ? afcm_conv2d_pack_weights2(dst, nullptr, w, dtype, cout, cin, ks, rows_pad, 0, stream)
                     : afcm_conv2d_pack_weights2(nullptr, dst, w, dtype, cout, cin, ks, 0, rows_pad, stream);
}

template <typename T>
static void launch_pack_bank(const PackBank& b, int blocks, int ks, int BK, hipStream_t st) {
    constexpr int BKT = ConvCfg<T>::BK;
    if constexpr (sizeof(T) == 2) {
        if (BK == 32) {
            hipLaunchKernelGGL((conv2d_pack_bank_kernel<T, 9, 32>), dim3(blocks), dim3(256), 0, st, b);
            return;
        }
    }
    if (ks == 3) hipLaunchKernelGGL((conv2d_pack_bank_kernel<T, 9, BKT>), dim3(blocks), dim3(256), 0, st, b);
    else hipLaunchKernelGGL((conv2d_pack_bank_kernel<T, 1, BKT>), dim3(blocks), dim3(256), 0, st, b);
}

extern "C" int afcm_conv2d_pack_bank(const afcm_pack_entry* entries, int32_t count, int32_t dtype, int32_t ks, void* stream) {
    AFCM_REQUIRE(entries != nullptr && count > 0 && count <= AFCM_PACK_MAX, "conv2d_pack_bank: 1..%d entries", AFCM_PACK_MAX);
    AFCM_REQUIRE(dtype == AFCM_F32 || dtype == AFCM_F16 || dtype == AFCM_BF16, "dtype must be float32, float16 or bfloat16");
    AFCM_REQUIRE(ks == 1 || ks == 3, "only 1x1 and 3x3 kernels are supported");
    const int BK = conv_bk(dtype, ks);
    const int ti = BK > 16 ? PackTile<32>::TI : 64, to = BK > 16 ? PackTile<32>::TO : 16;
    PackBank b;
    b.count = count;
    int tot = 0;
    for (int l = 0; l < count; l++) {
        const afcm_pack_entry& e = entries[l];
        AFCM_REQUIRE(e.w != nullptr && (e.dst_fwd != nullptr || e.dst_dgrad != nullptr) && e.cout > 0 && e.cin > 0, "conv2d_pack_bank: entry %d: null pointer or empty weights", l);
        AFCM_REQUIRE(e.dst_fwd == nullptr || (e.rows_pad_fwd >= e.cout && e.rows_pad_fwd % 64 == 0), "conv2d_pack_bank: entry %d: rows_pad must be a multiple of 64 covering the rows", l);
        AFCM_REQUIRE(e.dst_dgrad == nullptr || (e.rows_pad_dgrad >= e.cin && e.rows_pad_dgrad % 64 == 0), "conv2d_pack_bank: entry %d: rows_pad must be a multiple of 64 covering the rows", l);
        AFCM_REQUIRE((((uintptr_t)e.dst_fwd | (uintptr_t)e.dst_dgrad) & 31) == 0, "conv2d_pack_bank: entry %d: destinations must be 32-byte aligned", l);
        const int omax = e.dst_fwd ? e.rows_pad_fwd : round_up(e.cout, BK), imax = e.dst_dgrad ? e.rows_pad_dgrad : round_up(e.cin, BK);
        const int gx = cdiv(imax > e.cin ? imax : e.cin, ti), gy = cdiv(omax > e.cout ? omax : e.cout, to);
        b.e[l] = e;
        b.gx[l] = gx;
        b.blk[l] = tot;
        tot += gx * gy;
    }
    b.blk[count] = tot;
    hipStream_t st = (hipStream_t)stream;
    switch (dtype) {
        case AFCM_F32: launch_pack_bank<float>(b, tot, ks, BK, st); break;
        case AFCM_F16: launch_pack_bank<f16_t>(b, tot, ks, BK, st); break;
        default: launch_pack_bank<bf16_t>(b, tot, ks, BK, st); break;
    }
    return hip_status(hipGetLastError());
}

extern "C" int afcm_conv2d_stride2(void* y, const void* x, const void* wpacked, int32_t dtype, int32_t n, int32_t cin, int32_t cout, int32_t h,
                                   int32_t w, int32_t pad, int32_t rows_pad, void* stream) {
    AFCM_REQUIRE(y != nullptr && x != nullptr && wpacked != nullptr, "conv2d_stride2: null pointer");
    AFCM_REQUIRE(dtype == AFCM_F16 || dtype == AFCM_BF16, "conv2d_stride2: 16-bit activations only");
    AFCM_REQUIRE(n > 0 && cin > 0 && cout > 0 && h > 0 && w > 0 && (w % 2) == 0, "conv2d_stride2: empty x or odd width %d", w);
    AFCM_REQUIRE(pad >= 0 && pad <= 2, "padding must be in [0, k-1]");
    AFCM_REQUIRE(rows_pad >= cout && rows_pad % 128 == 0, "conv2d_stride2: rows_pad must be a multiple of 128 covering cout");
    AFCM_REQUIRE(h + 2 * pad >= 3 && w + 2 * pad >= 3, "output must be at least 1x1");
    ConvParams p;
    p.x = x; p.y = y; p.wp = wpacked; p.oscale = nullptr; p.obias = nullptr;
    p.N = n; p.Cin = cin; p.Cout = cout; p.H = h; p.W = w;
    p.P = (h + 2 * pad - 3) / 2 + 1; p.Q = (w + 2 * pad - 3) / 2 + 1;
    p.pad = pad;
    p.ldx = w; p.ldy = p.Q;
    choose_tile_s2(p.P, p.Q, &p.TH, &p.TW, &p.PWL);
    p.tilesX = cdiv(p.Q, p.TW); p.tilesY = cdiv(p.P, p.TH);
    p.magicTW = (unsigned)((0x100000000ull + (unsigned)p.TW - 1) / (unsigned)p.TW);
    p.magicTX = magic_u32((unsigned)p.tilesX); p.magicTY = magic_u32((unsigned)p.tilesY); p.magicN = magic_u32((unsigned)p.N); p.magicPC = magic_u32((unsigned)(p.PWL >> 2));
    p.Opad = rows_pad;
    p.nkc = cdiv(cin, afcm_conv2d_block_k(dtype));
    p.nkc_real = p.nkc; p.magicNK = 0; p.term_parts = 0; p.part_bytes = 0; p.last_part_bytes = 0; p.bound_a = p.bound_b = nullptr; p.total_blocks = 0; p.o_base = 0;
    const long long blocks = (long long)p.tilesX * p.tilesY * n * cdiv(cout, 128);
    AFCM_REQUIRE(blocks > 0 && blocks < (1ll << 31), "conv2d_stride2: grid of %lld blocks is out of range", blocks);
    AFCM_REQUIRE((long long)cin * h * w * 2ll < (1ll << 31), "conv2d_stride2: image out of range");
    if (dtype == AFCM_F16) hipLaunchKernelGGL((conv2d_fwd16s2_kernel<f16_t, 128>), dim3((unsigned)blocks), dim3(256), 0, (hipStream_t)stream, p);
    else hipLaunchKernelGGL((conv2d_fwd16s2_kernel<bf16_t, 128>), dim3((unsigned)blocks), dim3(256), 0, (hipStream_t)stream, p);
    return hip_status(hipGetLastError());
}

extern "C" int afcm_conv2d(void* y, const void* x, const void* wpacked, const float* oscale, const float* obias, int32_t dtype, int32_t n,
                           int32_t cin, int32_t cout, int32_t h, int32_t w, int32_t ks, int32_t pad, int32_t rows_pad, void* stream) {
    return afcm_conv2d_ld(y, x, wpacked, oscale, obias, dtype, n, cin, cout, h, w, ks, pad, rows_pad, 0, 0, stream);
}

extern "C" int afcm_conv2d_ld(void* y, const void* x, const void* wpacked, const float* oscale, const float* obias, int32_t dtype, int32_t n,
                              int32_t cin, int32_t cout, int32_t h, int32_t w, int32_t ks, int32_t pad, int32_t rows_pad, int32_t x_pitch,
                              int32_t y_pitch, void* stream) {
    AFCM_REQUIRE(y != nullptr && x != nullptr && wpacked != nullptr, "conv2d: null pointer");
    AFCM_REQUIRE(dtype == AFCM_F32 || dtype == AFCM_F16 || dtype == AFCM_BF16, "x must be float32, float16 or bfloat16");
    AFCM_REQUIRE(n > 0 && cin > 0 && cout > 0 && h > 0 && w > 0, "x is empty");
    AFCM_REQUIRE(ks == 1 || ks == 3, "only 1x1 and 3x3 kernels are supported");
    AFCM_REQUIRE(pad >= 0 && pad <= ks - 1, "padding must be in [0, k-1]");
    AFCM_REQUIRE(dtype == AFCM_F32 || (w % 2 == 0), "16-bit conv2d needs an even input width (got %d)", w);
    AFCM_REQUIRE(rows_pad >= cout && rows_pad % 64 == 0, "rows_pad must be a multiple of 64 covering cout");
    ConvParams p;
    p.x = x; p.y = y; p.wp = wpacked; p.oscale = oscale; p.obias = obias;
    p.N = n; p.Cin = cin; p.Cout = cout; p.H = h; p.W = w;
    p.P = h + 2 * pad - ks + 1; p.Q = w + 2 * pad - ks + 1;
    AFCM_REQUIRE(p.P >= 1 && p.Q >= 1, "output must be at least 1x1");
    p.pad = pad;
    p.ldx = x_pitch ? x_pitch : w; p.ldy = y_pitch ? y_pitch : p.Q;
    if (p.ldx != w || p.ldy != p.Q) {
        AFCM_REQUIRE(dtype != AFCM_F32 && ks == 3, "conv2d: row pitches need the 16-bit 3x3 kernel");
        AFCM_REQUIRE(p.ldx >= w && p.ldy >= p.Q && ((p.ldx | p.ldy) & 1) == 0, "conv2d: row pitches %d / %d must be even and cover the widths %d / %d", p.ldx, p.ldy, w, p.Q);
        AFCM_REQUIRE((long long)cout * p.P * p.ldy < (1ll << 30), "conv2d: pitched output image is out of range");
    }
    AFCM_REQUIRE(dtype == AFCM_F32 || ks != 3 || (long long)cout * p.P * p.ldy * 2 < (1ll << 30), "conv2d: 16-bit output image of %lld bytes is out of range (< 2^30)", (long long)cout * p.P * p.ldy * 2);
    if (dtype != AFCM_F32 && ks == 3 && cin <= 4 && cout <= 64) {
        return conv2d_direct_small_cin(x, y, wpacked, oscale, obias, dtype, n, cin, cout, h, w, pad, rows_pad, 32, p.ldx, p.ldy, (hipStream_t)stream);
    }
    choose_tile(p.P, p.Q, ks, &p.TH, &p.TW, &p.PWL, (dtype != AFCM_F32 && ks == 3) ? kPatchMaxX16 : kPatchMax);
    p.tilesX = cdiv(p.Q, p.TW); p.tilesY = cdiv(p.P, p.TH);
    p.magicTW = (unsigned)((0x100000000ull + (unsigned)p.TW - 1) / (unsigned)p.TW);
    p.magicTX = magic_u32((unsigned)p.tilesX); p.magicTY = magic_u32((unsigned)p.tilesY); p.magicN = magic_u32((unsigned)p.N); p.magicPC = magic_u32((unsigned)(p.PWL >> 2));
    p.Opad = rows_pad;
    p.nkc = cdiv(cin, conv_bk(dtype, ks));
    p.nkc_real = p.nkc; p.magicNK = 0; p.term_parts = 0; p.part_bytes = 0; p.last_part_bytes = 0; p.bound_a = p.bound_b = nullptr; p.total_blocks = 0; p.o_base = 0;
    hipStream_t st = (hipStream_t)stream;
    const bool small = (rows_pad % 128 != 0) || cout <= 64;
    if (dtype != AFCM_F32 && ks == 3 && cout > 64 && cout <= 96) {
        const long long blocks = (long long)p.tilesX * p.tilesY * p.N * cdiv(cout, 96);
        AFCM_REQUIRE(blocks > 0 && blocks < (1ll << 31), "conv2d: grid of %lld blocks is out of range", blocks);
        p.total_blocks = (int)blocks; p.o_base = 0;
        const dim3 g96((unsigned)conv_persistent_grid(blocks, 2));
        if (conv_fast_epilogue(p)) {
            if (dtype == AFCM_F16) hipLaunchKernelGGL((conv2d_fwd16x_kernel<f16_t, 96, false, true>), g96, dim3(256), 0, st, p);
            else hipLaunchKernelGGL((conv2d_fwd16x_kernel<bf16_t, 96, false, true>), g96, dim3(256), 0, st, p);
        } else if (dtype == AFCM_F16) hipLaunchKernelGGL((conv2d_fwd16x_kernel<f16_t, 96>), g96, dim3(256), 0, st, p);
        else hipLaunchKernelGGL((conv2d_fwd16x_kernel<bf16_t, 96>), g96, dim3(256), 0, st, p);
        return hip_status(hipGetLastError());
    }
    if (dtype != AFCM_F32 && ks == 3 && rows_pad % 128 == 64 && rows_pad > 128) {
        const int big = rows_pad / 128;
        const int rc = dtype == AFCM_F16 ? launch_conv<f16_t, 128>(p, ks, st, 0, big) : launch_conv<bf16_t, 128>(p, ks, st, 0, big);
        if (rc != AFCM_OK) return rc;
        return dtype == AFCM_F16 ? launch_conv<f16_t, 64>(p, ks, st, big * 128, 1) : launch_conv<bf16_t, 64>(p, ks, st, big * 128, 1);
    }
    switch (dtype) {
        case AFCM_F32: return small ? launch_conv<float, 64>(p, ks, st) : launch_conv<float, 128>(p, ks, st);
        case AFCM_F16: return small ? launch_conv<f16_t, 64>(p, ks, st) : launch_conv<f16_t, 128>(p, ks, st);
        default: return small ? launch_conv<bf16_t, 64>(p, ks, st) : launch_conv<bf16_t, 128>(p, ks, st);
    }
}


extern "C" int afcm_split16(void* parts, const float* x, const float* scale, const uint32_t* bound, int32_t dtype, int64_t planes, int32_t hw,
                            int32_t nparts, int64_t part_stride, void* stream) {
    AFCM_REQUIRE(parts != nullptr && x != nullptr && planes > 0 && hw > 0, "split16: empty input");
    AFCM_REQUIRE(dtype == AFCM_BF16 || dtype == AFCM_F16, "split16: parts are bfloat16 or float16");
    AFCM_REQUIRE(nparts == 2 || nparts == 3, "split16: 2 or 3 parts (got %d)", nparts);
    AFCM_REQUIRE(part_stride >= planes * (long long)hw && part_stride % 4 == 0, "split16: part stride %lld must cover the tensor and be a multiple of 4", (long long)part_stride);
    AFCM_REQUIRE(((uintptr_t)x & 15) == 0 && ((uintptr_t)parts & 7) == 0, "split16: x must be 16-byte, parts 8-byte aligned");
    long long blocks = (planes * ((hw + 3) >> 2) + 255) / 256;
    if (blocks > 4096) blocks = 4096;
    dim3 grid((unsigned)blocks), block(256);
    hipStream_t st = (hipStream_t)stream;
#define AFCM_SPLIT(T, K) hipLaunchKernelGGL((split16_kernel<T, K>), grid, block, 0, st, (T*)parts, x, scale, (const unsigned*)bound, (long long)planes, hw, (long long)part_stride)
    if (dtype == AFCM_BF16) { if (nparts == 2) AFCM_SPLIT(bf16_t, 2); else AFCM_SPLIT(bf16_t, 3); }
    else { if (nparts == 2) AFCM_SPLIT(f16_t, 2); else AFCM_SPLIT(f16_t, 3); }
#undef AFCM_SPLIT
    return hip_status(hipGetLastError());
}

extern "C" int afcm_amax_bits(uint32_t* out, const float* x, int64_t planes, int32_t hw, const float* scale, void* stream) {
    AFCM_REQUIRE(out != nullptr && x != nullptr && planes > 0 && hw > 0, "amax_bits: empty input");
    AFCM_REQUIRE(((uintptr_t)out & 3) == 0 && ((uintptr_t)x & 3) == 0, "amax_bits: misaligned pointer");
    long long blocks = (planes * hw / 16 + 255) / 256;
    blocks = blocks < 1 ? 1 : (blocks > 2048 ? 2048 : blocks);
    hipLaunchKernelGGL(amax_bits_kernel, dim3((unsigned)blocks), dim3(256), 0, (hipStream_t)stream, (unsigned*)out, x, (long long)planes, hw, scale);
    return hip_status(hipGetLastError());
}

extern "C" int afcm_plane_dot_parts(float* out, const void* parts, int64_t part_stride, int32_t nparts, const float* b, int32_t dtype, int64_t planes,
                                    int32_t hw, const uint32_t* bound, void* stream) {
    AFCM_REQUIRE(out != nullptr && parts != nullptr && b != nullptr && planes > 0 && hw > 0, "plane_dot_parts: empty input");
    AFCM_REQUIRE(dtype == AFCM_BF16 || dtype == AFCM_F16, "plane_dot_parts: parts are bfloat16 or float16");
    AFCM_REQUIRE(nparts >= 1 && nparts <= 3 && part_stride >= planes * (long long)hw, "plane_dot_parts: 1..3 parts, a stride covering the tensor");
    AFCM_REQUIRE(planes < (1ll << 31), "plane_dot_parts: too many planes");
    AFCM_REQUIRE(((uintptr_t)parts & 7) == 0 && ((uintptr_t)b & 15) == 0, "plane_dot_parts: parts must be 8-byte, b 16-byte aligned");
    hipStream_t st = (hipStream_t)stream;
    if (dtype == AFCM_BF16) hipLaunchKernelGGL((plane_dot_parts_kernel<bf16_t>), dim3((unsigned)planes), dim3(256), 0, st, out, (const bf16_t*)parts, (long long)part_stride, nparts, b, (long long)planes, hw, (const unsigned*)bound);
    else hipLaunchKernelGGL((plane_dot_parts_kernel<f16_t>), dim3((unsigned)planes), dim3(256), 0, st, out, (const f16_t*)parts, (long long)part_stride, nparts, b, (long long)planes, hw, (const unsigned*)bound);
    return hip_status(hipGetLastError());
}

extern "C" int afcm_unscale(float* t, int64_t numel, const uint32_t* bound_a, const uint32_t* bound_b, void* stream) {
    AFCM_REQUIRE(t != nullptr && numel > 0, "unscale: empty input");
    long long blocks = (numel + 255) / 256;
    if (blocks > 2048) blocks = 2048;
    hipLaunchKernelGGL(unscale_kernel, dim3((unsigned)blocks), dim3(256), 0, (hipStream_t)stream, t, (long long)numel, (const unsigned*)bound_a, (const unsigned*)bound_b);
    return hip_status(hipGetLastError());
}

extern "C" int afcm_conv2d_pack_split(void* dst, const float* w, const uint32_t* bound, int32_t dtype, int32_t cout, int32_t cin, int32_t mode,
                                      int32_t rows_pad, int32_t terms, uint32_t term_wparts, void* stream) {
    AFCM_REQUIRE(dst != nullptr && w != nullptr, "conv2d_pack_split: null pointer");
    AFCM_REQUIRE(dtype == AFCM_BF16 || dtype == AFCM_F16, "conv2d_pack_split: parts are bfloat16 or float16");
    AFCM_REQUIRE(mode == 0 || mode == 1, "mode must be 0 (forward) or 1 (data gradient)");
    AFCM_REQUIRE(terms >= 1 && terms <= 8 && cout > 0 && cin > 0, "conv2d_pack_split: 1..8 terms");
    const int rows = mode == 0 ? cout : cin, cols = mode == 0 ? cin : cout;
    AFCM_REQUIRE(rows_pad >= rows && rows_pad % 64 == 0, "rows_pad must be a multiple of 64 covering the rows");
    for (int t = 0; t < terms; t++) AFCM_REQUIRE(((term_wparts >> (4 * t)) & 15u) <= 2, "conv2d_pack_split: parts 0..2");
    const int BK = conv_bk(dtype, 3);
    const int nkc_real = cdiv(cols, BK);
    const long long total = (long long)terms * nkc_real * 9 * rows_pad * BK;
    long long blocks = (total + 255) / 256;
    if (blocks > 8192) blocks = 8192;
    hipStream_t st = (hipStream_t)stream;
    if (dtype == AFCM_BF16) hipLaunchKernelGGL((conv2d_pack_split_kernel<bf16_t>), dim3((unsigned)blocks), dim3(256), 0, st, (bf16_t*)dst, w, (const unsigned*)bound, cout, cin, rows, cols, rows_pad, nkc_real, terms, term_wparts, mode, BK);
    else hipLaunchKernelGGL((conv2d_pack_split_kernel<f16_t>), dim3((unsigned)blocks), dim3(256), 0, st, (f16_t*)dst, w, (const unsigned*)bound, cout, cin, rows, cols, rows_pad, nkc_real, terms, term_wparts, mode, BK);
    return hip_status(hipGetLastError());
}

extern "C" int afcm_conv2d_split(float* y, const void* x_parts, const void* wpacked, const float* oscale, const float* obias, int32_t dtype, int32_t n,
                                 int32_t cin, int32_t cout, int32_t h, int32_t w, int32_t pad, int32_t rows_pad, int32_t terms, uint32_t term_parts,
                                 int64_t part_stride, const uint32_t* bound_a, const uint32_t* bound_b, void* stream) {
    const int ks = 3;
    AFCM_REQUIRE(y != nullptr && x_parts != nullptr && wpacked != nullptr, "conv2d_split: null pointer");
    AFCM_REQUIRE(dtype == AFCM_BF16 || dtype == AFCM_F16, "conv2d_split: parts are bfloat16 or float16");
    AFCM_REQUIRE(n > 0 && cin > 0 && cout > 0 && h > 0 && w > 0, "x is empty");
    AFCM_REQUIRE(pad >= 0 && pad <= ks - 1, "padding must be in [0, k-1]");
    AFCM_REQUIRE(w % 2 == 0, "conv2d_split needs an even input width (got %d)", w);
    AFCM_REQUIRE(rows_pad >= cout && rows_pad % 64 == 0, "rows_pad must be a multiple of 64 covering cout");
    AFCM_REQUIRE(terms >= 1 && terms <= 8, "conv2d_split: 1..8 terms (got %d)", terms);
    int max_part = 0;
    for (int t = 0; t < terms; t++) max_part = std::max(max_part, (int)((term_parts >> (4 * t)) & 15u));
    AFCM_REQUIRE(max_part <= 2, "conv2d_split: parts 0..2");
    AFCM_REQUIRE(part_stride >= (long long)n * cin * h * w && (long long)max_part * part_stride * 2 < (1ll << 31) - (long long)cin * h * w * 2,
                 "conv2d_split: part stride %lld out of range", (long long)part_stride);
    ConvParams p;
    p.x = x_parts; p.y = y; p.wp = wpacked; p.oscale = oscale; p.obias = obias;
    p.N = n; p.Cin = cin; p.Cout = cout; p.H = h; p.W = w;
    p.P = h + 2 * pad - ks + 1; p.Q = w + 2 * pad - ks + 1;
    AFCM_REQUIRE(p.P >= 1 && p.Q >= 1, "output must be at least 1x1");
    p.pad = pad;
    p.ldx = w; p.ldy = p.Q;
    choose_tile(p.P, p.Q, ks, &p.TH, &p.TW, &p.PWL, kPatchMaxX16);
    p.tilesX = cdiv(p.Q, p.TW); p.tilesY = cdiv(p.P, p.TH);
    p.magicTW = (unsigned)((0x100000000ull + (unsigned)p.TW - 1) / (unsigned)p.TW);
    p.magicTX = magic_u32((unsigned)p.tilesX); p.magicTY = magic_u32((unsigned)p.tilesY); p.magicN = magic_u32((unsigned)p.N); p.magicPC = magic_u32((unsigned)(p.PWL >> 2));
    p.Opad = rows_pad;
    p.nkc_real = cdiv(cin, conv_bk(dtype, 3));
    p.nkc = terms * p.nkc_real;
    p.magicNK = magic_u32((unsigned)p.nkc_real);
    p.term_parts = term_parts;
    p.part_bytes = (int)(part_stride * 2);
    p.last_part_bytes = max_part * p.part_bytes;
    p.bound_a = (const unsigned*)bound_a; p.bound_b = (const unsigned*)bound_b;
    const bool small = (rows_pad % 128 != 0) || cout <= 64;
    const long long blocks = (long long)p.tilesX * p.tilesY * p.N * cdiv(p.Cout, small ? 64 : 128);
    AFCM_REQUIRE(blocks > 0 && blocks < (1ll << 31), "conv2d_split: grid of %lld blocks is out of range", blocks);
    const dim3 block(256);
    hipStream_t st = (hipStream_t)stream;
    p.total_blocks = (int)blocks; p.o_base = 0;
    const dim3 pgrid(small ? (unsigned)conv_persistent_grid(blocks, 3) : (unsigned)blocks);
    if (dtype == AFCM_BF16) {
        if (small) hipLaunchKernelGGL((conv2d_fwd16x_kernel<bf16_t, 64, true>), pgrid, block, 0, st, p);
        else hipLaunchKernelGGL((conv2d_fwd16x_kernel<bf16_t, 128, true>), pgrid, block, 0, st, p);
    } else {
        if (small) hipLaunchKernelGGL((conv2d_fwd16x_kernel<f16_t, 64, true>), pgrid, block, 0, st, p);
        else hipLaunchKernelGGL((conv2d_fwd16x_kernel<f16_t, 128, true>), pgrid, block, 0, st, p);
    }
    return hip_status(hipGetLastError());
}

static int wgrad_rows_per_step(int dtype) { return dtype == AFCM_F32 ? 1 : 2; }

static int wgrad_splits(int n, int cout, int cin, int p_rows) {
    const int tiles = cdiv(cout, 64) * cdiv(cin, 64);
    const long long ksteps = (long long)n * p_rows;
    int s = 256 / tiles;
    if (s > ksteps) s = (int)ksteps;
    return s < 1 ? 1 : s;
}

extern "C" int afcm_conv2d_wgrad_splits(int32_t n, int32_t cout, int32_t cin, int32_t p_rows) {
    return wgrad_splits(n, cout, cin, p_rows);
}

extern "C" int afcm_conv2d_wgrad(float* dw, float* workspace, const void* dy, const void* x, int32_t dtype, int32_t n, int32_t cin,
                                 int32_t cout, int32_t h, int32_t w, int32_t ks, int32_t pad, void* stream) {
    return afcm_conv2d_wgrad_ld(dw, workspace, dy, x, dtype, n, cin, cout, h, w, ks, pad, 0, 0, stream);
}

static int wgrad_impl(float* dw, float* workspace, const void* dy, const void* x, int32_t dtype, int32_t n, int32_t cin,
                      int32_t cout, int32_t h, int32_t w, int32_t ks, int32_t pad, int32_t dy_pitch, int32_t x_pitch, float* dots, const float* wref, void* stream) {
    AFCM_REQUIRE(dw != nullptr && workspace != nullptr && dy != nullptr && x != nullptr, "conv2d_wgrad: null pointer");
    AFCM_REQUIRE(dtype == AFCM_F32 || dtype == AFCM_F16 || dtype == AFCM_BF16, "x must be float32, float16 or bfloat16");
    AFCM_REQUIRE(ks == 1 || ks == 3, "only 1x1 and 3x3 kernels are supported");
    AFCM_REQUIRE(pad >= 0 && pad <= ks - 1, "padding must be in [0, k-1]");
    WgradParams p;
    p.dy = dy; p.x = x; p.part = workspace;
    p.N = n; p.O = cout; p.I = cin; p.H = h; p.W = w; p.pad = pad;
    p.P = h + 2 * pad - ks + 1; p.Q = w + 2 * pad - ks + 1;
    AFCM_REQUIRE(p.P >= 1 && p.Q >= 1, "output must be at least 1x1");
    AFCM_REQUIRE(dtype == AFCM_F32 || (w % 2 == 0 && p.Q % 2 == 0), "16-bit conv2d_wgrad needs even widths (got %d, %d)", w, p.Q);
    p.lddy = dy_pitch ? dy_pitch : p.Q; p.ldx = x_pitch ? x_pitch : w;
    const bool pitched = p.lddy != p.Q || p.ldx != w;
    AFCM_REQUIRE(!pitched || (p.lddy >= p.Q && p.ldx >= w && ((p.lddy | p.ldx) & 1) == 0), "conv2d_wgrad: row pitches %d / %d must be even and cover the widths %d / %d", p.lddy, p.ldx, p.Q, w);
    const int R = wgrad_rows_per_step(dtype);
    p.qchunks = cdiv(p.Q, kWgKQ);
    p.rowgroups = cdiv(p.P, R);
    const long long ksteps = (long long)n * p.rowgroups * p.qchunks;
    const bool granule = (ks == 3 && pad == 2) || (ks == 1 && pad == 0);
    p.fo = cdiv(cout, 64); p.fi = cdiv(cin, 64);
    p.splits = p.splits_p = wgrad_splits(n, cout, cin, p.P);
    if (p.splits > ksteps) p.splits = (int)ksteps;
    if (p.splits_p > ksteps) p.splits_p = (int)ksteps;
    p.steps_per_split = (int)((ksteps + p.splits - 1) / p.splits);
    p.steps_per_split_p = (int)((ksteps + p.splits_p - 1) / p.splits_p);
    p.splits_img = 0;
    if (dots != nullptr) {
        if (!(dtype != AFCM_F32 && granule) || n > 64 || p.splits % n != 0 || p.splits / n < 1) return AFCM_E_NOKERNEL;
        AFCM_REQUIRE(wref != nullptr, "conv2d_wgrad_dots: the weight tensor the dot products are taken with is missing");
        p.splits_img = p.splits / n;
        const long long per_img = (long long)p.rowgroups * p.qchunks;
        p.steps_per_split = p.steps_per_split_p = (int)((per_img + p.splits_img - 1) / p.splits_img);
    }
    const long long n_full = (long long)p.fo * p.fi;
    const long long blocks = n_full * p.splits + ((long long)cdiv(cout, 64) * cdiv(cin, 64) - n_full) * p.splits_p;
    dim3 grid((unsigned)blocks), block(512);
    hipStream_t st = (hipStream_t)stream;
#define AFCM_WG(T, R) do { if (ks == 3 && (pad & 1) == 0) hipLaunchKernelGGL((conv2d_wgrad_kernel<T, 3, R, 0>), grid, block, 0, st, p); \
                           else if (ks == 3) hipLaunchKernelGGL((conv2d_wgrad_kernel<T, 3, R, 1>), grid, block, 0, st, p); \
                           else hipLaunchKernelGGL((conv2d_wgrad_kernel<T, 1, R, 0>), grid, block, 0, st, p); } while (0)
#define AFCM_WG16(T) do { constexpr int NB = 3; \
                           if (ks == 3 && (pad & 1) == 0) hipLaunchKernelGGL((conv2d_wgrad16_kernel<T, 3, 0, NB>), grid, block, 0, st, p); \
                           else if (ks == 3) hipLaunchKernelGGL((conv2d_wgrad16_kernel<T, 3, 1, NB>), grid, block, 0, st, p); \
                           else hipLaunchKernelGGL((conv2d_wgrad16_kernel<T, 1, 0, NB>), grid, block, 0, st, p); } while (0)
#define AFCM_WG16G_(T, X) do { constexpr int NB = kWgradRing; \
                            if (small && ks == 3) hipLaunchKernelGGL((conv2d_wgrad16g_kernel<T, 3, NB, true, X>), grid, block, 0, st, p); \
                            else if (small) hipLaunchKernelGGL((conv2d_wgrad16g_kernel<T, 1, NB, true, X>), grid, block, 0, st, p); \
                            else if (ks == 3) hipLaunchKernelGGL((conv2d_wgrad16g_kernel<T, 3, NB, false, X>), grid, block, 0, st, p); \
                            else hipLaunchKernelGGL((conv2d_wgrad16g_kernel<T, 1, NB, false, X>), grid, block, 0, st, p); } while (0)
    const int q_last = p.Q % 64;
    const bool wg_x16 = !(q_last > 32 && q_last <= 48);
#define AFCM_WG16G(T) do { if (wg_x16) AFCM_WG16G_(T, true); else AFCM_WG16G_(T, false); } while (0)
    const bool small = (long long)n * cout * p.P * p.lddy * 2 < (1ll << 31) - 65536 &&
                       (long long)n * cin * h * p.ldx * 2 < (1ll << 31) - 65536;
    AFCM_REQUIRE(!pitched || (dtype != AFCM_F32 && granule), "conv2d_wgrad: row pitches need the 16-bit granule kernel (3x3 pad 2 or 1x1 pad 0)");
    switch (dtype) {
        case AFCM_F32: AFCM_WG(float, 1); break;
        case AFCM_F16: if (granule) AFCM_WG16G(f16_t); else AFCM_WG16(f16_t); break;
        default: if (granule) AFCM_WG16G(bf16_t); else AFCM_WG16(bf16_t); break;
    }
#undef AFCM_WG16G
#undef AFCM_WG16G_
#undef AFCM_WG16
#undef AFCM_WG
    int rc = hip_status(hipGetLastError());
    if (rc != AFCM_OK) return rc;
    const long long numel = (long long)cout * cin * ks * ks;
    if (p.splits_img > 0) {
        const dim3 rgrid((unsigned)cin), rblock(1024);
#define AFCM_RD(T) do { if (ks == 3) hipLaunchKernelGGL((wgrad_reduce_dots_kernel<T, 9>), rgrid, rblock, 0, st, dw, dots, (const float*)workspace, wref, n, cout, cin, p.splits_img); \
                        else hipLaunchKernelGGL((wgrad_reduce_dots_kernel<T, 1>), rgrid, rblock, 0, st, dw, dots, (const float*)workspace, wref, n, cout, cin, p.splits_img); } while (0)
        if (dtype == AFCM_F16) AFCM_RD(f16_t); else AFCM_RD(bf16_t);
#undef AFCM_RD
        return hip_status(hipGetLastError());
    }
    const WgradSlabs slabs{cin, ks * ks, p.fo, p.fi, p.splits, p.splits_p};
    long long rb = (numel + 255) / 256;
    if (rb > 2048) rb = 2048;
    if ((numel & 3) == 0 && (((uintptr_t)dw | (uintptr_t)workspace) & 15) == 0) {
        const long long n4 = numel / 4;
        if (p.splits >= 64) hipLaunchKernelGGL(wgrad_reduce4_kernel<16>, dim3((unsigned)cdiv(n4, 16)), dim3(256), 0, st, dw, (const float*)workspace, n4, slabs);
        else if (p.splits >= 8) hipLaunchKernelGGL(wgrad_reduce4_kernel<64>, dim3((unsigned)cdiv(n4, 64)), dim3(256), 0, st, dw, (const float*)workspace, n4, slabs);
        else hipLaunchKernelGGL(wgrad_reduce4_kernel<256>, dim3((unsigned)cdiv(n4, 256)), dim3(256), 0, st, dw, (const float*)workspace, n4, slabs);
    } else {
        hipLaunchKernelGGL(wgrad_reduce_kernel, dim3((unsigned)rb), dim3(256), 0, st, dw, (const float*)workspace, numel, slabs);
    }
    return hip_status(hipGetLastError());
}

extern "C" int afcm_conv2d_wgrad_ld(float* dw, float* workspace, const void* dy, const void* x, int32_t dtype, int32_t n, int32_t cin,
                                    int32_t cout, int32_t h, int32_t w, int32_t ks, int32_t pad, int32_t dy_pitch, int32_t x_pitch, void* stream) {
    return wgrad_impl(dw, workspace, dy, x, dtype, n, cin, cout, h, w, ks, pad, dy_pitch, x_pitch, nullptr, nullptr, stream);
}

extern "C" int afcm_conv2d_wgrad_dots_ld(float* dw, float* dots, float* workspace, const void* dy, const void* x, const float* wref, int32_t dtype,
                                         int32_t n, int32_t cin, int32_t cout, int32_t h, int32_t w, int32_t ks, int32_t pad, int32_t dy_pitch,
                                         int32_t x_pitch, void* stream) {
    AFCM_REQUIRE(dots != nullptr, "conv2d_wgrad_dots: dots must be non-null");
    return wgrad_impl(dw, workspace, dy, x, dtype, n, cin, cout, h, w, ks, pad, dy_pitch, x_pitch, dots, wref, stream);
}

extern "C" int afcm_scale_planes(void* y, const void* x, const float* scale, int32_t dtype_in, int32_t dtype_out, int64_t planes,
                                 int32_t hw, void* stream) {
    AFCM_REQUIRE(y != nullptr && x != nullptr && planes > 0 && hw > 0, "scale_planes: empty input");
    long long blocks = (planes * ((hw + 3) >> 2) + 255) / 256;
    if (blocks > 2048) blocks = 2048;
    dim3 grid((unsigned)blocks), block(256);
    hipStream_t st = (hipStream_t)stream;
#define AFCM_SP(TI, TO) hipLaunchKernelGGL((scale_planes_kernel<TI, TO>), grid, block, 0, st, (TO*)y, (const TI*)x, scale, (long long)planes, hw)
    if (dtype_in == AFCM_F32 && dtype_out == AFCM_F32) AFCM_SP(float, float);
    else if (dtype_in == AFCM_F32 && dtype_out == AFCM_BF16) AFCM_SP(float, bf16_t);
    else if (dtype_in == AFCM_F32 && dtype_out == AFCM_F16) AFCM_SP(float, f16_t);
    else if (dtype_in == AFCM_BF16 && dtype_out == AFCM_BF16) AFCM_SP(bf16_t, bf16_t);
    else if (dtype_in == AFCM_F16 && dtype_out == AFCM_F16) AFCM_SP(f16_t, f16_t);
    else if (dtype_in == AFCM_BF16 && dtype_out == AFCM_F32) AFCM_SP(bf16_t, float);
    else if (dtype_in == AFCM_F16 && dtype_out == AFCM_F32) AFCM_SP(f16_t, float);
    else { set_error("scale_planes: unsupported dtype pair %d -> %d", dtype_in, dtype_out); return AFCM_E_INVALID; }
#undef AFCM_SP
    return hip_status(hipGetLastError());
}

extern "C" int afcm_axpy_planes(void* y, const void* a, const void* b, const float* scale, int32_t dtype, int64_t planes, int32_t hw, void* stream) {
    AFCM_REQUIRE(y != nullptr && a != nullptr && b != nullptr && planes > 0 && hw > 0, "axpy_planes: empty input");
    AFCM_REQUIRE(dtype == AFCM_F16 || dtype == AFCM_BF16, "axpy_planes: 16-bit tensors only");
    if ((hw & 7) != 0 || ((((uintptr_t)y | (uintptr_t)a | (uintptr_t)b)) & 15) != 0) return AFCM_E_NOKERNEL;
    const int per = hw >> 3;
    const dim3 grid((unsigned)((per + 1023) / 1024), (unsigned)(planes < 65535 ? planes : 65535));
    hipStream_t st = (hipStream_t)stream;
    if (dtype == AFCM_BF16) hipLaunchKernelGGL((axpy_planes_kernel<bf16_t>), grid, dim3(256), 0, st, (bf16_t*)y, (const bf16_t*)a, (const bf16_t*)b, scale, (long long)planes, hw);
    else hipLaunchKernelGGL((axpy_planes_kernel<f16_t>), grid, dim3(256), 0, st, (f16_t*)y, (const f16_t*)a, (const f16_t*)b, scale, (long long)planes, hw);
    return hip_status(hipGetLastError());
}

extern "C" int afcm_plane_dot(float* out, const void* a, const void* b, int32_t dtype, int64_t planes, int32_t hw, void* stream) {
    AFCM_REQUIRE(out != nullptr && a != nullptr && planes > 0 && hw > 0, "plane_dot: empty input");
    AFCM_REQUIRE(planes < (1ll << 31), "plane_dot: too many planes");
    AFCM_REQUIRE((((uintptr_t)a | (uintptr_t)b) & 15) == 0, "plane_dot: operands must be 16-byte aligned");
    hipStream_t st = (hipStream_t)stream;
    const int esize = dtype == AFCM_F32 ? 4 : 2;
    const bool per_wave = (long long)hw * esize <= 16384;
    dim3 grid((unsigned)(per_wave ? (planes + 3) / 4 : planes)), block(256);
#define AFCM_PD(T) do { \
        if (per_wave) hipLaunchKernelGGL((plane_dot_wave_kernel<T>), grid, block, 0, st, out, (const T*)a, (const T*)b, (long long)planes, hw); \
        else hipLaunchKernelGGL((plane_dot_kernel<T>), grid, block, 0, st, out, (const T*)a, (const T*)b, (long long)planes, hw); } while (0)
    switch (dtype) {
        case AFCM_F32: AFCM_PD(float); break;
        case AFCM_F16: AFCM_PD(f16_t); break;
        case AFCM_BF16: AFCM_PD(bf16_t); break;
        default: set_error("plane_dot: bad dtype"); return AFCM_E_INVALID;
    }
#undef AFCM_PD
    return hip_status(hipGetLastError());
}

static int plane_dot_rows(float* out, const void* a, const void* b, int32_t dtype, int64_t planes, int32_t h, int32_t w,
                          int32_t a_pitch, int32_t b_pitch, const PlaneGate& gate, void* stream) {
    AFCM_REQUIRE(out != nullptr && a != nullptr && planes > 0 && h > 0 && w > 0, "plane_dot: empty input");
    AFCM_REQUIRE(planes < (1ll << 31), "plane_dot: too many planes");
    const int esize = dtype == AFCM_F32 ? 4 : 2;
    const int lda = a_pitch ? a_pitch : w, ldb = b_pitch ? b_pitch : w;
    AFCM_REQUIRE(lda >= w && ldb >= w, "plane_dot: row pitches %d / %d are below the width %d", lda, ldb, w);
    AFCM_REQUIRE(w >= 16 / esize, "plane_dot: rows of %d elements are shorter than one 16-byte vector", w);
    AFCM_REQUIRE((((uintptr_t)a | (uintptr_t)b) & 3) == 0 && (esize == 4 || ((w | lda | ldb) & 1) == 0), "plane_dot: rows must start on 4-byte boundaries");
    AFCM_REQUIRE((long long)h * (lda > ldb ? lda : ldb) < (1ll << 31) / 16, "plane_dot: plane is out of range");
    hipStream_t st = (hipStream_t)stream;
    const bool per_wave = (long long)h * w * esize <= 16384;
    dim3 grid((unsigned)(per_wave ? (planes + 3) / 4 : planes)), block(256);
#define AFCM_PDR(T) do { \
        if (per_wave) hipLaunchKernelGGL((plane_dot_rows_kernel<T, true>), grid, block, 0, st, out, (const T*)a, (const T*)b, (long long)planes, h, w, lda, ldb, gate); \
        else hipLaunchKernelGGL((plane_dot_rows_kernel<T, false>), grid, block, 0, st, out, (const T*)a, (const T*)b, (long long)planes, h, w, lda, ldb, gate); } while (0)
    switch (dtype) {
        case AFCM_F32: AFCM_PDR(float); break;
        case AFCM_F16: AFCM_PDR(f16_t); break;
        case AFCM_BF16: AFCM_PDR(bf16_t); break;
        default: set_error("plane_dot: bad dtype"); return AFCM_E_INVALID;
    }
#undef AFCM_PDR
    return hip_status(hipGetLastError());
}

extern "C" int afcm_plane_dot_ld(float* out, const void* a, const void* b, int32_t dtype, int64_t planes, int32_t h, int32_t w,
                                 int32_t a_pitch, int32_t b_pitch, void* stream) {
    return plane_dot_rows(out, a, b, dtype, planes, h, w, a_pitch, b_pitch, PlaneGate{nullptr, 0, nullptr, nullptr, nullptr, nullptr}, stream);
}

extern "C" int afcm_plane_dot_gated_ld(float* out, const void* a, const void* b, int32_t dtype, int64_t planes, int32_t h, int32_t w,
                                       int32_t a_pitch, int32_t b_pitch, const int32_t* flags, int32_t slots, const float* out_scale,
                                       const float* gz, const float* next_scale, const float* gskip, void* stream) {
    AFCM_REQUIRE(flags != nullptr && slots > 0 && out_scale != nullptr && gz != nullptr && b != nullptr, "plane_dot_gated: null pointer");
    return plane_dot_rows(out, a, b, dtype, planes, h, w, a_pitch, b_pitch, PlaneGate{flags, slots, out_scale, gz, next_scale, gskip}, stream);
}
```

### include/afcm_hip.h

```cpp
#ifndef AFCM_HIP_H
#define AFCM_HIP_H

#include <stdint.h>

#ifdef __cplusplus
extern "C" {
#endif

#define AFCM_ABI_VERSION 13

enum { AFCM_F32 = 0, AFCM_F16 = 1, AFCM_BF16 = 2 };
enum { AFCM_OK = 0, AFCM_E_NOKERNEL = -1, AFCM_E_INVALID = -2 };
enum { AFCM_SIGNS_NONE = 0, AFCM_SIGNS_WRITE = 1, AFCM_SIGNS_READ = 2 };

int afcm_abi_version(void);
const char* afcm_last_error(void);
int afcm_noop(void* stream);

typedef struct afcm_filtered_lrelu_args {
    const void* x;
    void*       y;
    const void* b;
    uint8_t*    signs;
    const float* fu;
    const float* fd;
    int32_t dtype;
    int32_t n, c, xh, xw, yh, yw;
    int32_t fuw, fuh, fdw, fdh;
    int32_t up, down;
    int32_t px0, px1, py0, py1;
    int32_t sx, sy;
    int32_t sh, swb;
    float   gain, slope, clamp;
    int32_t flip_filter;
    int32_t sign_mode;
    void*   workspace;
    int32_t sign_layout;
    int32_t plane_sum_slots;
    float*  plane_sum;
    const float* oscale;
    const void*  skip;
    const float* oscale2;
    int32_t x_pitch, y_pitch, skip_pitch;
    int32_t row_pitch_ok;
    int32_t* clamp_flags;
} afcm_filtered_lrelu_args;

int afcm_filtered_lrelu_shapes(afcm_filtered_lrelu_args* a);
int afcm_filtered_lrelu(const afcm_filtered_lrelu_args* a, void* stream);

int64_t afcm_filtered_lrelu_workspace_bytes(void);
int afcm_filtered_lrelu_prepare(const afcm_filtered_lrelu_args* a, void* stream);

int afcm_filtered_lrelu_act(void* x, uint8_t* signs, int32_t dtype, int32_t n, int32_t c, int32_t h, int32_t w,
                            int32_t sh, int32_t swb, int32_t sx, int32_t sy, float gain, float slope, float clamp,
                            int32_t sign_mode, void* stream);

int afcm_upfirdn2d(void* y, const void* x, const float* f, int32_t dtype, int32_t n, int32_t c, int32_t xh, int32_t xw,
                   int32_t yh, int32_t yw, int32_t fh, int32_t fw, int32_t upx, int32_t upy, int32_t downx, int32_t downy,
                   int32_t padx0, int32_t pady0, int32_t flip, float gain, void* stream);

int afcm_bias_act(void* y, const void* x, const void* b, const void* xref, const void* yref, const void* dy,
                  int32_t dtype, int64_t numel, int64_t inner, int32_t nb, int32_t grad, int32_t act, float alpha,
                  float gain, float clamp, void* stream);



int afcm_conv2d_block_k(int32_t dtype);
int afcm_conv2d_block_k_ks(int32_t dtype, int32_t ks);

int afcm_conv2d_pack_weights(void* dst, const float* w, int32_t dtype, int32_t cout, int32_t cin, int32_t ks,
                             int32_t mode, int32_t rows_pad, void* stream);

int afcm_conv2d_pack_weights2(void* dst_fwd, void* dst_dgrad, const float* w, int32_t dtype, int32_t cout, int32_t cin, int32_t ks,
                              int32_t rows_pad_fwd, int32_t rows_pad_dgrad, void* stream);
int afcm_conv2d_pack_weights_bk(void* dst, const float* w, int32_t dtype, int32_t cout, int32_t cin, int32_t ks, int32_t mode,
                                int32_t rows_pad, int32_t block_k, void* stream);

int afcm_conv2d(void* y, const void* x, const void* wpacked, const float* oscale, const float* obias, int32_t dtype, int32_t n,
                int32_t cin, int32_t cout, int32_t h, int32_t w, int32_t ks, int32_t pad, int32_t rows_pad, void* stream);
int afcm_conv2d_ld(void* y, const void* x, const void* wpacked, const float* oscale, const float* obias, int32_t dtype, int32_t n,
                   int32_t cin, int32_t cout, int32_t h, int32_t w, int32_t ks, int32_t pad, int32_t rows_pad, int32_t x_pitch,
                   int32_t y_pitch, void* stream);

int afcm_conv2d_wgrad_splits(int32_t n, int32_t cout, int32_t cin, int32_t p_rows);
int afcm_conv2d_wgrad(float* dw, float* workspace, const void* dy, const void* x, int32_t dtype, int32_t n, int32_t cin,
                      int32_t cout, int32_t h, int32_t w, int32_t ks, int32_t pad, void* stream);
int afcm_conv2d_wgrad_ld(float* dw, float* workspace, const void* dy, const void* x, int32_t dtype, int32_t n, int32_t cin,
                         int32_t cout, int32_t h, int32_t w, int32_t ks, int32_t pad, int32_t dy_pitch, int32_t x_pitch, void* stream);
int afcm_conv2d_wgrad_dots_ld(float* dw, float* dots, float* workspace, const void* dy, const void* x, const float* wref, int32_t dtype, int32_t n,
                              int32_t cin, int32_t cout, int32_t h, int32_t w, int32_t ks, int32_t pad, int32_t dy_pitch, int32_t x_pitch,
                              void* stream);

int afcm_scale_planes(void* y, const void* x, const float* scale, int32_t dtype_in, int32_t dtype_out, int64_t planes,
                      int32_t hw, void* stream);

int afcm_plane_dot(float* out, const void* a, const void* b, int32_t dtype, int64_t planes, int32_t hw, void* stream);
int afcm_plane_dot_ld(float* out, const void* a, const void* b, int32_t dtype, int64_t planes, int32_t h, int32_t w,
                      int32_t a_pitch, int32_t b_pitch, void* stream);
int afcm_plane_dot_gated_ld(float* out, const void* a, const void* b, int32_t dtype, int64_t planes, int32_t h, int32_t w,
                            int32_t a_pitch, int32_t b_pitch, const int32_t* flags, int32_t slots, const float* out_scale,
                            const float* gz, const float* next_scale, const float* gskip, void* stream);

int afcm_weight_norm_fwd(float* w_hat, float* wsq, float* scale, const float* w, int32_t cout, int32_t cin, int32_t kk, void* stream);
int afcm_weight_norm_bwd(float* dw, const float* g_hat, const float* g_wsq, const float* w_hat, const float* scale, int32_t cout,
                         int32_t cin, int32_t kk, void* stream);
int afcm_style_coefs_fwd(float* s_eff, float* d, float* r, const float* t, const float* wsq, const float* magnitude, int32_t n, int32_t cin,
                         int32_t cout, int32_t demodulate, void* stream);
int afcm_style_coefs_bwd(float* dt, float* g_wsq, float* workspace, const float* g_s, const float* g_d, const float* t, const float* d,
                         const float* wsq, const float* magnitude, const float* r, int32_t n, int32_t cin, int32_t cout, int32_t demodulate,
                         void* stream);

int afcm_layer_bwd_coefs(float* db, float* d_next, float* d_out, const float* psum, int32_t slots, const float* out_scale,
                         const float* next_scale, const float* bias, const float* gz, const float* dysy, int32_t n, int32_t cout,
                         void* stream);

typedef struct afcm_adam_entry {
    void*   p;
    void*   g;
    void*   m;
    void*   v;
    int64_t numel;
    int64_t chunk0;
} afcm_adam_entry;
int32_t afcm_adam_chunk_elems(void);
int afcm_adam_multi(const afcm_adam_entry* table, int32_t n, int64_t total_chunks, float step_size, float beta1, float beta2,
                    float one_minus_beta1, float one_minus_beta2, float bias_correction2_sqrt, float eps, float grad_scale, int32_t scrub, float posinf, float neginf,
                    int32_t write_grad, void* stream);
int afcm_adam_multi_capturable(const afcm_adam_entry* table_dev, int32_t n, int64_t total_chunks, float* step_dev, float lr, float beta1, float beta2,
                               float eps, float grad_scale, int32_t scrub, float posinf, float neginf, int32_t write_grad, void* stream);

#define AFCM_AFFINE_MAX 16
typedef struct afcm_affine_bank {
    int32_t layers, n, kw, kg;
    int64_t w_stride_n, w_stride_l;
    const float* w;
    const float* g;
    const float* weight[AFCM_AFFINE_MAX];
    const float* bias[AFCM_AFFINE_MAX];
    int32_t cout[AFCM_AFFINE_MAX];
    int32_t w_index[AFCM_AFFINE_MAX];
    float alpha[AFCM_AFFINE_MAX], beta[AFCM_AFFINE_MAX];
} afcm_affine_bank;
int64_t afcm_affine_bank_workspace_bytes(const afcm_affine_bank* a);
int afcm_affine_bank_fwd(const afcm_affine_bank* a, float* const* y, void* stream);
int afcm_affine_bank_bwd(const afcm_affine_bank* a, const float* const* dy, float* const* dweight, float* const* dbias, float* dws, float* dg,
                         void* workspace, void* stream);

#define AFCM_MODULATION_MAX 16
typedef struct afcm_modulation_layer {
    int32_t cout, cin, kk, demodulate;
    const float* w;
    const float* t;
    const float* magnitude;
    float* w_hat;
    float* wsq;
    float* scale;
    float* s_eff;
    float* d;
    float* r;
    const float* g_hat;
    const float* g_s;
    const float* g_d;
    float* dw;
    float* dt;
    float* workspace;
} afcm_modulation_layer;
int64_t afcm_modulation_bank_workspace_floats(int32_t n, int32_t cin, int32_t cout, int32_t demodulate);
int afcm_modulation_bank_fwd(const afcm_modulation_layer* layers, int32_t count, int32_t n, void* stream);
int afcm_modulation_bank_bwd(const afcm_modulation_layer* layers, int32_t count, int32_t n, void* stream);

#define AFCM_PACK_MAX 32
typedef struct afcm_pack_entry {
    void* dst_fwd;
    void* dst_dgrad;
    const float* w;
    int32_t cout, cin, rows_pad_fwd, rows_pad_dgrad;
} afcm_pack_entry;
int afcm_conv2d_pack_bank(const afcm_pack_entry* entries, int32_t count, int32_t dtype, int32_t ks, void* stream);

int afcm_amax_bits(uint32_t* out, const float* x, int64_t planes, int32_t hw, const float* scale, void* stream);
int afcm_split16(void* parts, const float* x, const float* scale, const uint32_t* bound, int32_t dtype, int64_t planes, int32_t hw,
                 int32_t nparts, int64_t part_stride, void* stream);
int afcm_unscale(float* t, int64_t numel, const uint32_t* bound_a, const uint32_t* bound_b, void* stream);
int afcm_plane_dot_parts(float* out, const void* parts, int64_t part_stride, int32_t nparts, const float* b, int32_t dtype, int64_t planes,
                         int32_t hw, const uint32_t* bound, void* stream);
int afcm_conv2d_pack_split(void* dst, const float* w, const uint32_t* bound, int32_t dtype, int32_t cout, int32_t cin, int32_t mode,
                           int32_t rows_pad, int32_t terms, uint32_t term_wparts, void* stream);
int afcm_conv2d_split(float* y, const void* x_parts, const void* wpacked, const float* oscale, const float* obias, int32_t dtype, int32_t n,
                      int32_t cin, int32_t cout, int32_t h, int32_t w, int32_t pad, int32_t rows_pad, int32_t terms, uint32_t term_parts,
                      int64_t part_stride, const uint32_t* bound_a, const uint32_t* bound_b, void* stream);

int afcm_conv2d_stride2(void* y, const void* x, const void* wpacked, int32_t dtype, int32_t n, int32_t cin, int32_t cout, int32_t h, int32_t w,
                        int32_t pad, int32_t rows_pad, void* stream);

int afcm_pool_blocks_fwd(float* y, const void* x, int32_t dtype, int64_t planes, int32_t h, int32_t w, void* stream);
int afcm_pool_blocks_bwd(void* dx, const float* gy, int32_t dtype, int64_t planes, int32_t h, int32_t w, void* stream);

int afcm_l1_partials(float* partials, const float* a, const float* b, int64_t numel, int32_t blocks, float weight, void* stream);
int afcm_l1_grad(float* ga, const float* a, const float* b, const float* gout, int64_t numel, float weight, void* stream);

int afcm_axpy_planes(void* y, const void* a, const void* b, const float* scale, int32_t dtype, int64_t planes, int32_t hw, void* stream);

int afcm_fc_act_fwd(float* y, const float* x, const float* w, const float* b, int32_t n, int32_t cin, int32_t cout, float alpha, float beta,
                    int32_t act, void* stream);
int afcm_fc_act_bwd(float* dx, float* dw, float* db, const float* gy, const float* y, const float* x, const float* w, int32_t n, int32_t cin,
                    int32_t cout, float alpha, float beta, int32_t act, void* stream);
int afcm_mapping_input_fwd(float* x0, const float* z, const float* c, const float* ew, const float* eb, int32_t n, int32_t zdim, int32_t cdim,
                           int32_t wdim, float alpha, float beta, void* stream);
int64_t afcm_mapping_input_bwd_workspace_bytes(int32_t n, int32_t wdim);
int afcm_mapping_input_bwd(float* dew, float* deb, const float* gx0, const float* c, const float* ew, const float* eb, int32_t n, int32_t zdim,
                           int32_t cdim, int32_t wdim, float alpha, float beta, void* workspace, void* stream);

#ifdef __cplusplus
}
#endif
#endif
```

Measured before the change: 486.4 images/sec.

## Add cost-model tile planner with 128/192/256-pixel conv tiles

Templates the 16-bit 3x3 forward conv kernel on the number of 16-pixel fragments per warp (4, 6 or 8), so tiles can hold 128, 192 or 256 pixels. A host-side cost model estimates wave quantization and tail rounds over 2 blocks per CU and picks a smaller tile when it cuts modeled cost by a margin, aiming to fill the GPU on small spatial layers. This adds more template instantiations and a heuristic plan that can misjudge per-tile efficiency. It also exposes plan and explicit-tile entry points.

```diff
diff --git a/afcm_amd/_lib.py b/afcm_amd/_lib.py
--- a/afcm_amd/_lib.py
+++ b/afcm_amd/_lib.py
@@ -85,6 +85,9 @@
     'afcm_conv2d_pack_weights2': (C.c_int, [_vp, _vp, _vp, _i32, _i32, _i32, _i32, _i32, _i32, _vp]),
     'afcm_conv2d': (C.c_int, [_vp, _vp, _vp, _vp, _vp, _i32, _i32, _i32, _i32, _i32, _i32, _i32, _i32, _i32, _vp]),
     'afcm_conv2d_ld': (C.c_int, [_vp, _vp, _vp, _vp, _vp, _i32, _i32, _i32, _i32, _i32, _i32, _i32, _i32, _i32, _i32, _i32, _vp]),
+    'afcm_conv2d_plan': (C.c_int, [_i32, _i32, _i32, _i32, _i32, _i32, _i32, _i32, _i32, _i32, _vp, _vp]),
+    'afcm_conv2d_tile_ld': (C.c_int, [_vp, _vp, _vp, _vp, _vp, _i32, _i32, _i32, _i32, _i32, _i32, _i32, _i32, _i32, _i32, _i32, _i32, _i32,
+                                      _vp]),
     'afcm_conv2d_wgrad_splits': (C.c_int, [_i32, _i32, _i32, _i32]),
     'afcm_conv2d_wgrad': (C.c_int, [_vp, _vp, _vp, _vp, _i32, _i32, _i32, _i32, _i32, _i32, _i32, _i32, _vp]),
     'afcm_conv2d_wgrad_ld': (C.c_int, [_vp, _vp, _vp, _vp, _i32, _i32, _i32, _i32, _i32, _i32, _i32, _i32, _i32, _i32, _vp]),
@@ -94,6 +97,8 @@
     'afcm_plane_dot_ld': (C.c_int, [_vp, _vp, _vp, _i32, _i64, _i32, _i32, _i32, _i32, _vp]),
     'afcm_split16': (C.c_int, [_vp, _vp, _vp, _vp, _i32, _i64, _i32, _i32, _i64, _vp]),
     'afcm_conv2d_split': (C.c_int, [_vp, _vp, _vp, _vp, _vp, _i32, _i32, _i32, _i32, _i32, _i32, _i32, _i32, _i32, C.c_uint32, _i64, _vp, _vp, _vp]),
+    'afcm_conv2d_split_tile': (C.c_int, [_vp, _vp, _vp, _vp, _vp, _i32, _i32, _i32, _i32, _i32, _i32, _i32, _i32, _i32, C.c_uint32, _i64, _vp,
+                                         _vp, _i32, _i32, _i32, _vp]),
     'afcm_amax_bits': (C.c_int, [_vp, _vp, _i64, _i32, _vp, _vp]),
     'afcm_unscale': (C.c_int, [_vp, _i64, _vp, _vp, _vp]),
     'afcm_plane_dot_parts': (C.c_int, [_vp, _vp, _i64, _i32, _vp, _i32, _i64, _i32, _vp, _vp]),
diff --git a/afcm_amd/csrc/conv2d.hip b/afcm_amd/csrc/conv2d.hip
--- a/afcm_amd/csrc/conv2d.hip
+++ b/afcm_amd/csrc/conv2d.hip
@@ -309,12 +309,16 @@
     }
 }
 
-template <typename T, int BM_O, bool SPLIT = false, bool FASTEPI = false>
+template <typename T, int BM_O, bool SPLIT = false, bool FASTEPI = false, int NT = 8>
 __global__ __launch_bounds__(256, 2) void conv2d_fwd16x_kernel(ConvParams p) {
     static_assert(sizeof(T) == 2, "16-bit types only");
     static_assert(!(SPLIT && FASTEPI), "the fp32-output epilogue has no fast form");
+    static_assert(NT == 8 || NT == 6 || NT == 4, "tiles of 256, 192 or 128 pixels");
     typedef typename std::conditional<SPLIT, float, T>::type TO;
-    constexpr int KS = 3, KK = 9, BK = 32, MO = BM_O / 32, NT = 8, BRING = MO == 4 ? 4 : 3;
+    constexpr int KS = 3, KK = 9, BK = 32, MO = BM_O / 32, BRING = MO == 4 ? 4 : 3;
+    constexpr int PXW = 16 * NT;
+    constexpr int MSTEPS = NT > 4 ? NT - 4 : 1;
+    static_assert(BRING <= NT, "the ring's first fragments are blocks of tap 0");
     constexpr int ARING = MO == 2 ? 6 : 9;
     static_assert((KK * MO) % ARING == 0 && ARING >= 2 * MO, "static slots; a tap's fragments and the next tap's are live together");
     constexpr int PLANE_B = kPlaneX16 * 16;
@@ -429,7 +433,7 @@
             const unsigned lanepart = (unsigned)((lane_o & 15) * 16 + (lane_o >> 4) * PLANE_B);
 #pragma unroll
             for (int ti = 0; ti < NT; ti++) {
-                const int b16 = wpx * 128 + ti * 16;
+                const int b16 = wpx * PXW + ti * 16;
                 int py = (int)__umulhi((unsigned)b16, p.magicTW), px = b16 - py * p.TW;
                 if (b16 >= p.TH * p.TW) { py = 0; px = 0; }
                 bbyte[ti] = lanepart + (unsigned)((py * PWL + px + xoff) * 16 + buf * BUF_B);
@@ -438,7 +442,7 @@
         }
 #pragma unroll
         for (int ti = 0; ti < NT; ti++) {
-            const int j = wpx * 128 + ti * 16 + (lane_o & 15);
+            const int j = wpx * PXW + ti * 16 + (lane_o & 15);
             int py = (int)__umulhi((unsigned)j, p.magicTW), px = j - py * p.TW;
             if (j >= p.TH * p.TW) { py = 0; px = 0; }
             bbyte[ti] = (unsigned)((py * PWL + px + xoff) * 16 + (lane_o >> 4) * PLANE_B + buf * BUF_B);
@@ -511,10 +515,14 @@
                     if (tap == 0 && ti == 0) issue_patch(preg, knext, more, 0);
                     if (tap == 5 && ti == 0) issue_patch(preg, knext, more, 1);
                     if (tap == 4 || tap == 8) {
-                        if (ti < 4) { mask_ch(preg, 2 * ti); mask_ch(preg, 2 * ti + 1); }
-                        else write_px(preg, ti - 4, nxt_b + (tap == 8 ? 2 * PLANE_B : 0));
+#pragma unroll
+                        for (int m = 0; m < 4; m++)
+                            if (m * MSTEPS / 4 == ti) { mask_ch(preg, 2 * m); mask_ch(preg, 2 * m + 1); }
+                        if (ti >= NT - 4) write_px(preg, ti - (NT - 4), nxt_b + (tap == 8 ? 2 * PLANE_B : 0));
                     }
-                    if (tap == 8 && ti >= 4) { bbyte[2 * (ti - 4)] += bufstep; bbyte[2 * (ti - 4) + 1] += bufstep; }
+                    if (tap == 8 && ti >= NT / 2) {
+                        bbyte[2 * (ti - NT / 2)] += bufstep; bbyte[2 * (ti - NT / 2) + 1] += bufstep;
+                    }
                     if (ti == NT - 1) {
 #pragma unroll
                         for (int mo = 0; mo < MO; mo++) {
@@ -564,10 +572,10 @@
             unsigned wr_off[2];
 #pragma unroll
             for (int k = 0; k < 2; k++) wr_off[k] = (unsigned)(c16e * EROW + (((4 * k + ge) ^ ((c16e >> 1) & 7)) << 3));
-            unsigned gbyte[8], gfullm = 0, slow_any = 0;
-#pragma unroll
-            for (int it = 0; it < (FASTEPI ? 0 : 8); it++) {
-                const int j0 = wpx * 128 + (2 * it + hh) * 8;
+            unsigned gbyte[NT], gfullm = 0, slow_any = 0;
+#pragma unroll
+            for (int it = 0; it < (FASTEPI ? 0 : NT); it++) {
+                const int j0 = wpx * PXW + (2 * it + hh) * 8;
                 const int gpy = (int)__umulhi((unsigned)j0, p.magicTW), gpx = j0 - gpy * p.TW;
                 const int gy = y0 + gpy, gx = x0 + gpx;
                 const bool in_tile = j0 < p.TH * p.TW && gy < p.P;
@@ -584,13 +592,15 @@
                 const int o = rowbase + chalf * 16 + i16;
                 const unsigned obyte = (o < p.Cout && mi * 32 + chalf * 16 < BM_O / 2) ? (unsigned)(o * pq * 2) : kOOut;
 #pragma unroll
-                for (int half = 0; half < 2; half++) {
+                for (int half = 0; half < (NT + 3) / 4; half++) {
+                    constexpr int NB = 4;
+                    const int nb = NT - 4 * half < NB ? NT - 4 * half : NB;
 #pragma unroll
                     for (int k = 0; k < 2; k++) {
                         const int mo = 2 * mi + k;
                         if (mo >= MO) continue;
 #pragma unroll
-                        for (int t4 = 0; t4 < 4; t4++) {
+                        for (int t4 = 0; t4 < nb; t4++) {
                             const int ti = 4 * half + t4;
                             uint2 w;
                             w.x = pack2<T>(acc[mo][ti][0] * sc[mo][0] + ob[mo][0], acc[mo][ti][1] * sc[mo][1] + ob[mo][1]);
@@ -599,14 +609,14 @@
                         }
                     }
 #pragma unroll
-                    for (int i4 = 0; i4 < 4; i4++) {
+                    for (int i4 = 0; i4 < nb; i4++) {
                         const int it = 4 * half + i4;
                         union { s16x4 v[2]; eu32x4 q; } u;
 #pragma unroll
                         for (int r = 0; r < 2; r++)
                             u.v[r] = __builtin_amdgcn_ds_read_tr16_b64_v4i16((__attribute__((address_space(3))) s16x4*)(ebuf + i4 * (16 * EROW) + rd_off[r]));
                         if constexpr (FASTEPI) {
-                            const int b16 = wpx * 128 + 16 * it;
+                            const int b16 = wpx * PXW + 16 * it;
                             const int gpy = (int)__umulhi((unsigned)b16, p.magicTW), gpxs = b16 - gpy * p.TW;
                             const int gy = y0 + gpy, gxs = x0 + gpxs;
                             if (b16 < p.TH * p.TW && gy < p.P && gxs < p.Q) {
@@ -622,7 +632,7 @@
                             if (!full) {
 #pragma unroll
                                 for (int w2 = 0; w2 < 4; w2++) {
-                                    const int j = wpx * 128 + (2 * it + hh) * 8 + 2 * w2;
+                                    const int j = wpx * PXW + (2 * it + hh) * 8 + 2 * w2;
                                     const int py = (int)__umulhi((unsigned)j, p.magicTW), px = j - py * p.TW;
                                     const bool ok = j < p.TH * p.TW && y0 + py < p.P && x0 + px < p.Q;
                                     __builtin_amdgcn_raw_buffer_store_b32(u.q[w2], yrs, ok ? obyte + (unsigned)(((y0 + py) * p.ldy + x0 + px) * 2) : kGOut, 0, 0);
@@ -637,7 +647,7 @@
             int poff[NT];
 #pragma unroll
             for (int ti = 0; ti < NT; ti++) {
-                const int j = wpx * 128 + ti * 16 + c16e;
+                const int j = wpx * PXW + ti * 16 + c16e;
                 const int py = (int)__umulhi((unsigned)j, p.magicTW), px = j - py * p.TW;
                 poff[ti] = (j < p.TH * p.TW && y0 + py < p.P && x0 + px < p.Q) ? (y0 + py) * p.ldy + x0 + px : -1;
             }
@@ -2561,7 +2571,7 @@
     }
 }
 
-static int conv_persistent_grid(long long items, int per_cu) {
+static int conv_device_cus() {
     static int cus[16] = {0};
     int dev = 0;
     (void)hipGetDevice(&dev);
@@ -2570,16 +2580,102 @@
         if (hipDeviceGetAttribute(&n, hipDeviceAttributeMultiprocessorCount, dev) != hipSuccess || n <= 0) n = 256;
         if (dev >= 0 && dev < 16) cus[dev] = n;
     }
-    const long long slots = (long long)round_up(n * per_cu, 8);
+    return n;
+}
+
+static int conv_persistent_grid(long long items, int per_cu) {
+    const long long slots = (long long)round_up(conv_device_cus() * per_cu, 8);
     return (int)(items < slots ? items : slots);
+}
+
+constexpr double kPlanTile[3] = {0.8, 0.95, 1.0};
+constexpr double kPlanTail = 0.2;
+constexpr double kPlanMargin = 0.05;
+constexpr double kPlanGranule = 0.03;
+
+struct ConvPlan { int nt, th, tw, pwl; double cost, cost_base; };
+struct ConvLaunchShape { int row_blocks, mo; };
+
+static int conv16_launch_shapes(int cout, int rows_pad, bool split, ConvLaunchShape (&ls)[2]) {
+    const bool small = (rows_pad % 128 != 0) || cout <= 64;
+    if (!split && cout > 64 && cout <= 96) { ls[0] = {cdiv(cout, 96), 3}; return 1; }
+    if (!split && rows_pad % 128 == 64 && rows_pad > 128) { ls[0] = {rows_pad / 128, 4}; ls[1] = {1, 2}; return 2; }
+    ls[0] = small ? ConvLaunchShape{cdiv(cout, 64), 2} : ConvLaunchShape{cdiv(cout, 128), 4};
+    return 1;
+}
+
+static double conv_plan_cost(int P, int Q, int n, int nt, int th, int tw, const ConvLaunchShape* ls, int nls, int cus) {
+    const long long tiles = (long long)cdiv(P, th) * cdiv(Q, tw) * n;
+    const long long slots = 2ll * cus;
+    double c = 0;
+    for (int l = 0; l < nls; l++) {
+        const long long w = tiles * ls[l].row_blocks;
+        const long long full = w / slots, rest = w % slots;
+        const double rounds = (double)full + (rest ? kPlanTail + (1.0 - kPlanTail) * (double)rest / (double)slots : 0.0);
+        c += rounds * ls[l].mo / 4.0 * kPlanTile[nt / 2 - 2];
+    }
+    return c * ((tw & 7) ? 1.0 + kPlanGranule : 1.0);
+}
+
+static int conv_tile_height(int P, int nt, int tw) {
+    int th = std::min(32 * nt / tw, P);
+    while (th >= 1 && (th + 2) * round_up(tw + 3, 4) > kPatchMaxX16) th--;
+    return th;
+}
+
+static ConvPlan conv_plan(int P, int Q, int n, int cout, int rows_pad, bool split, int cus) {
+    ConvLaunchShape ls[2];
+    const int nls = conv16_launch_shapes(cout, rows_pad, split, ls);
+    ConvPlan base;
+    base.nt = 8;
+    choose_tile(P, Q, 3, &base.th, &base.tw, &base.pwl, kPatchMaxX16);
+    base.cost = base.cost_base = conv_plan_cost(P, Q, n, 8, base.th, base.tw, ls, nls, cus);
+    ConvPlan best = base;
+    for (int nt = 8; nt >= 4; nt -= 2)
+        for (int tw = 2; tw <= 128; tw += 2) {
+            const int th = conv_tile_height(P, nt, tw);
+            if (th < 1) continue;
+            const double c = conv_plan_cost(P, Q, n, nt, th, tw, ls, nls, cus);
+            if (c < best.cost * (1.0 - 1e-9)) best = ConvPlan{nt, th, tw, round_up(tw + 3, 4), c, base.cost_base};
+        }
+    return best.cost < base.cost_base * (1.0 - kPlanMargin) ? best : base;
+}
+
+static void conv_set_tile(ConvParams& p, int th, int tw, int pwl) {
+    p.TH = th; p.TW = tw; p.PWL = pwl;
+    p.tilesX = cdiv(p.Q, p.TW); p.tilesY = cdiv(p.P, p.TH);
+    p.magicTW = (unsigned)((0x100000000ull + (unsigned)p.TW - 1) / (unsigned)p.TW);
+    p.magicTX = magic_u32((unsigned)p.tilesX); p.magicTY = magic_u32((unsigned)p.tilesY); p.magicN = magic_u32((unsigned)p.N); p.magicPC = magic_u32((unsigned)(p.PWL >> 2));
+}
+
+static const char* conv_tile_invalid(int nt, int th, int tw) {
+    if (nt != 4 && nt != 6 && nt != 8) return "nt must be 4, 6 or 8";
+    if (th < 1 || tw < 2 || (tw & 1) || tw > 128) return "tile width must be even in [2, 128], height >= 1";
+    if (th * tw > 32 * nt) return "tile holds more than 32 nt pixels";
+    if ((th + 2) * round_up(tw + 3, 4) > kPatchMaxX16) return "tile patch exceeds the LDS plane";
+    return nullptr;
 }
 
 static bool conv_fast_epilogue(const ConvParams& p) {
     return (p.TW & 15) == 0 && (p.ldy & 7) == 0 && (p.Q & 1) == 0;
 }
 
+template <typename T, int BM_O, bool SPLIT, int NT>
+static void launch_fwd16x_nt(const ConvParams& p, dim3 grid, hipStream_t st) {
+    if constexpr (!SPLIT) {
+        if (conv_fast_epilogue(p)) { hipLaunchKernelGGL((conv2d_fwd16x_kernel<T, BM_O, false, true, NT>), grid, dim3(256), 0, st, p); return; }
+    }
+    hipLaunchKernelGGL((conv2d_fwd16x_kernel<T, BM_O, SPLIT, false, NT>), grid, dim3(256), 0, st, p);
+}
+template <typename T, int BM_O, bool SPLIT>
+static void launch_fwd16x(const ConvParams& p, int nt, dim3 grid, hipStream_t st) {
+    if (nt == 4) launch_fwd16x_nt<T, BM_O, SPLIT, 4>(p, grid, st);
+    else if (nt == 6) launch_fwd16x_nt<T, BM_O, SPLIT, 6>(p, grid, st);
+    else launch_fwd16x_nt<T, BM_O, SPLIT, 8>(p, grid, st);
+}
+
 template <typename T, int BM_O>
-static int launch_conv(ConvParams p, int ks, hipStream_t st, int o_base = 0, int row_blocks = 0) {
+static int launch_conv(ConvParams p, int ks, hipStream_t st, int o_base = 0, int row_blocks = 0, int nt = 8) {
     const long long blocks = (long long)p.tilesX * p.tilesY * p.N * (row_blocks ? row_blocks : cdiv(p.Cout, BM_O));
     p.o_base = o_base;
     AFCM_REQUIRE(blocks > 0 && blocks < (1ll << 31), "conv2d: grid of %lld blocks is out of range", blocks);
@@ -2588,8 +2684,7 @@
     if constexpr (sizeof(T) == 2) {
         if (ks == 3) {
             const dim3 g16 = BM_O == 64 ? dim3((unsigned)conv_persistent_grid(blocks, 3)) : grid;
-            if (conv_fast_epilogue(p)) hipLaunchKernelGGL((conv2d_fwd16x_kernel<T, BM_O, false, true>), g16, block, 0, st, p);
-            else hipLaunchKernelGGL((conv2d_fwd16x_kernel<T, BM_O>), g16, block, 0, st, p);
+            launch_fwd16x<T, BM_O, false>(p, nt, g16, st);
             return hip_status(hipGetLastError());
         }
     }
@@ -2741,9 +2836,9 @@
     return afcm_conv2d_ld(y, x, wpacked, oscale, obias, dtype, n, cin, cout, h, w, ks, pad, rows_pad, 0, 0, stream);
 }
 
-extern "C" int afcm_conv2d_ld(void* y, const void* x, const void* wpacked, const float* oscale, const float* obias, int32_t dtype, int32_t n,
-                              int32_t cin, int32_t cout, int32_t h, int32_t w, int32_t ks, int32_t pad, int32_t rows_pad, int32_t x_pitch,
-                              int32_t y_pitch, void* stream) {
+static int conv2d_ld_impl(void* y, const void* x, const void* wpacked, const float* oscale, const float* obias, int32_t dtype, int32_t n,
+                          int32_t cin, int32_t cout, int32_t h, int32_t w, int32_t ks, int32_t pad, int32_t rows_pad, int32_t x_pitch,
+                          int32_t y_pitch, const int* tile, void* stream) {
     AFCM_REQUIRE(y != nullptr && x != nullptr && wpacked != nullptr, "conv2d: null pointer");
     AFCM_REQUIRE(dtype == AFCM_F32 || dtype == AFCM_F16 || dtype == AFCM_BF16, "x must be float32, float16 or bfloat16");
     AFCM_REQUIRE(n > 0 && cin > 0 && cout > 0 && h > 0 && w > 0, "x is empty");
@@ -2765,12 +2860,25 @@
     }
     AFCM_REQUIRE(dtype == AFCM_F32 || ks != 3 || (long long)cout * p.P * p.ldy * 2 < (1ll << 30), "conv2d: 16-bit output image of %lld bytes is out of range (< 2^30)", (long long)cout * p.P * p.ldy * 2);
     if (dtype != AFCM_F32 && ks == 3 && cin <= 4 && cout <= 64) {
+        AFCM_REQUIRE(tile == nullptr, "conv2d: the small-cin kernel (cin <= 4, cout <= 64) has no tile plan");
         return conv2d_direct_small_cin(x, y, wpacked, oscale, obias, dtype, n, cin, cout, h, w, pad, rows_pad, 32, p.ldx, p.ldy, (hipStream_t)stream);
     }
-    choose_tile(p.P, p.Q, ks, &p.TH, &p.TW, &p.PWL, (dtype != AFCM_F32 && ks == 3) ? kPatchMaxX16 : kPatchMax);
-    p.tilesX = cdiv(p.Q, p.TW); p.tilesY = cdiv(p.P, p.TH);
-    p.magicTW = (unsigned)((0x100000000ull + (unsigned)p.TW - 1) / (unsigned)p.TW);
-    p.magicTX = magic_u32((unsigned)p.tilesX); p.magicTY = magic_u32((unsigned)p.tilesY); p.magicN = magic_u32((unsigned)p.N); p.magicPC = magic_u32((unsigned)(p.PWL >> 2));
+    const bool x16 = dtype != AFCM_F32 && ks == 3;
+    int nt = 8;
+    if (!x16) {
+        AFCM_REQUIRE(tile == nullptr, "conv2d: tile plans are for the 16-bit 3x3 kernel");
+        choose_tile(p.P, p.Q, ks, &p.TH, &p.TW, &p.PWL, kPatchMax);
+        conv_set_tile(p, p.TH, p.TW, p.PWL);
+    } else if (tile != nullptr) {
+        const char* bad = conv_tile_invalid(tile[0], tile[1], tile[2]);
+        AFCM_REQUIRE(bad == nullptr, "conv2d: %s (nt %d, tile %d x %d)", bad ? bad : "", tile[0], tile[1], tile[2]);
+        nt = tile[0];
+        conv_set_tile(p, tile[1], tile[2], round_up(tile[2] + 3, 4));
+    } else {
+        const ConvPlan pl = conv_plan(p.P, p.Q, n, cout, rows_pad, false, conv_device_cus());
+        nt = pl.nt;
+        conv_set_tile(p, pl.th, pl.tw, pl.pwl);
+    }
     p.Opad = rows_pad;
     p.nkc = cdiv(cin, conv_bk(dtype, ks));
     p.nkc_real = p.nkc; p.magicNK = 0; p.term_parts = 0; p.part_bytes = 0; p.last_part_bytes = 0; p.bound_a = p.bound_b = nullptr; p.total_blocks = 0; p.o_base = 0;
@@ -2781,24 +2889,51 @@
         AFCM_REQUIRE(blocks > 0 && blocks < (1ll << 31), "conv2d: grid of %lld blocks is out of range", blocks);
         p.total_blocks = (int)blocks; p.o_base = 0;
         const dim3 g96((unsigned)conv_persistent_grid(blocks, 2));
-        if (conv_fast_epilogue(p)) {
-            if (dtype == AFCM_F16) hipLaunchKernelGGL((conv2d_fwd16x_kernel<f16_t, 96, false, true>), g96, dim3(256), 0, st, p);
-            else hipLaunchKernelGGL((conv2d_fwd16x_kernel<bf16_t, 96, false, true>), g96, dim3(256), 0, st, p);
-        } else if (dtype == AFCM_F16) hipLaunchKernelGGL((conv2d_fwd16x_kernel<f16_t, 96>), g96, dim3(256), 0, st, p);
-        else hipLaunchKernelGGL((conv2d_fwd16x_kernel<bf16_t, 96>), g96, dim3(256), 0, st, p);
+        if (dtype == AFCM_F16) launch_fwd16x<f16_t, 96, false>(p, nt, g96, st);
+        else launch_fwd16x<bf16_t, 96, false>(p, nt, g96, st);
         return hip_status(hipGetLastError());
     }
     if (dtype != AFCM_F32 && ks == 3 && rows_pad % 128 == 64 && rows_pad > 128) {
         const int big = rows_pad / 128;
-        const int rc = dtype == AFCM_F16 ? launch_conv<f16_t, 128>(p, ks, st, 0, big) : launch_conv<bf16_t, 128>(p, ks, st, 0, big);
+        const int rc = dtype == AFCM_F16 ? launch_conv<f16_t, 128>(p, ks, st, 0, big, nt) : launch_conv<bf16_t, 128>(p, ks, st, 0, big, nt);
         if (rc != AFCM_OK) return rc;
-        return dtype == AFCM_F16 ? launch_conv<f16_t, 64>(p, ks, st, big * 128, 1) : launch_conv<bf16_t, 64>(p, ks, st, big * 128, 1);
+        return dtype == AFCM_F16 ? launch_conv<f16_t, 64>(p, ks, st, big * 128, 1, nt) : launch_conv<bf16_t, 64>(p, ks, st, big * 128, 1, nt);
     }
     switch (dtype) {
         case AFCM_F32: return small ? launch_conv<float, 64>(p, ks, st) : launch_conv<float, 128>(p, ks, st);
-        case AFCM_F16: return small ? launch_conv<f16_t, 64>(p, ks, st) : launch_conv<f16_t, 128>(p, ks, st);
-        default: return small ? launch_conv<bf16_t, 64>(p, ks, st) : launch_conv<bf16_t, 128>(p, ks, st);
-    }
+        case AFCM_F16: return small ? launch_conv<f16_t, 64>(p, ks, st, 0, 0, nt) : launch_conv<f16_t, 128>(p, ks, st, 0, 0, nt);
+        default: return small ? launch_conv<bf16_t, 64>(p, ks, st, 0, 0, nt) : launch_conv<bf16_t, 128>(p, ks, st, 0, 0, nt);
+    }
+}
+
+extern "C" int afcm_conv2d_ld(void* y, const void* x, const void* wpacked, const float* oscale, const float* obias, int32_t dtype, int32_t n,
+                              int32_t cin, int32_t cout, int32_t h, int32_t w, int32_t ks, int32_t pad, int32_t rows_pad, int32_t x_pitch,
+                              int32_t y_pitch, void* stream) {
+    return conv2d_ld_impl(y, x, wpacked, oscale, obias, dtype, n, cin, cout, h, w, ks, pad, rows_pad, x_pitch, y_pitch, nullptr, stream);
+}
+
+extern "C" int afcm_conv2d_tile_ld(void* y, const void* x, const void* wpacked, const float* oscale, const float* obias, int32_t dtype, int32_t n,
+                                   int32_t cin, int32_t cout, int32_t h, int32_t w, int32_t pad, int32_t rows_pad, int32_t x_pitch, int32_t y_pitch,
+                                   int32_t nt, int32_t th, int32_t tw, void* stream) {
+    AFCM_REQUIRE(dtype == AFCM_F16 || dtype == AFCM_BF16, "conv2d_tile_ld: 16-bit activations only");
+    const int tile[3] = {nt, th, tw};
+    return conv2d_ld_impl(y, x, wpacked, oscale, obias, dtype, n, cin, cout, h, w, 3, pad, rows_pad, x_pitch, y_pitch, tile, stream);
+}
+
+extern "C" int afcm_conv2d_plan(int32_t dtype, int32_t n, int32_t cin, int32_t cout, int32_t h, int32_t w, int32_t pad, int32_t rows_pad,
+                                int32_t split, int32_t cus, int32_t* plan, float* cost) {
+    AFCM_REQUIRE(plan != nullptr, "conv2d_plan: null plan");
+    AFCM_REQUIRE(dtype == AFCM_F16 || dtype == AFCM_BF16, "conv2d_plan: the plan is for 16-bit (or split) 3x3 convolutions");
+    AFCM_REQUIRE(n > 0 && cin > 0 && cout > 0 && pad >= 0 && pad <= 2 && h + 2 * pad >= 3 && w + 2 * pad >= 3, "conv2d_plan: bad shape");
+    AFCM_REQUIRE(rows_pad >= cout && rows_pad % 64 == 0, "rows_pad must be a multiple of 64 covering cout");
+    AFCM_REQUIRE(cus >= 0, "conv2d_plan: negative CU count");
+    if (!split && cin <= 4 && cout <= 64) return AFCM_E_NOKERNEL;
+    const ConvPlan pl = conv_plan(h + 2 * pad - 2, w + 2 * pad - 2, n, cout, rows_pad, split != 0, cus ? cus : conv_device_cus());
+    ConvPlan base;
+    choose_tile(h + 2 * pad - 2, w + 2 * pad - 2, 3, &base.th, &base.tw, &base.pwl, kPatchMaxX16);
+    plan[0] = pl.nt; plan[1] = pl.th; plan[2] = pl.tw; plan[3] = 8; plan[4] = base.th; plan[5] = base.tw;
+    if (cost) { cost[0] = (float)pl.cost; cost[1] = (float)pl.cost_base; }
+    return AFCM_OK;
 }
 
 
@@ -2870,9 +3005,9 @@
     return hip_status(hipGetLastError());
 }
 
-extern "C" int afcm_conv2d_split(float* y, const void* x_parts, const void* wpacked, const float* oscale, const float* obias, int32_t dtype, int32_t n,
-                                 int32_t cin, int32_t cout, int32_t h, int32_t w, int32_t pad, int32_t rows_pad, int32_t terms, uint32_t term_parts,
-                                 int64_t part_stride, const uint32_t* bound_a, const uint32_t* bound_b, void* stream) {
+static int conv2d_split_impl(float* y, const void* x_parts, const void* wpacked, const float* oscale, const float* obias, int32_t dtype, int32_t n,
+                             int32_t cin, int32_t cout, int32_t h, int32_t w, int32_t pad, int32_t rows_pad, int32_t terms, uint32_t term_parts,
+                             int64_t part_stride, const uint32_t* bound_a, const uint32_t* bound_b, const int* tile, void* stream) {
     const int ks = 3;
     AFCM_REQUIRE(y != nullptr && x_parts != nullptr && wpacked != nullptr, "conv2d_split: null pointer");
     AFCM_REQUIRE(dtype == AFCM_BF16 || dtype == AFCM_F16, "conv2d_split: parts are bfloat16 or float16");
@@ -2893,10 +3028,17 @@
     AFCM_REQUIRE(p.P >= 1 && p.Q >= 1, "output must be at least 1x1");
     p.pad = pad;
     p.ldx = w; p.ldy = p.Q;
-    choose_tile(p.P, p.Q, ks, &p.TH, &p.TW, &p.PWL, kPatchMaxX16);
-    p.tilesX = cdiv(p.Q, p.TW); p.tilesY = cdiv(p.P, p.TH);
-    p.magicTW = (unsigned)((0x100000000ull + (unsigned)p.TW - 1) / (unsigned)p.TW);
-    p.magicTX = magic_u32((unsigned)p.tilesX); p.magicTY = magic_u32((unsigned)p.tilesY); p.magicN = magic_u32((unsigned)p.N); p.magicPC = magic_u32((unsigned)(p.PWL >> 2));
+    int nt;
+    if (tile != nullptr) {
+        const char* bad = conv_tile_invalid(tile[0], tile[1], tile[2]);
+        AFCM_REQUIRE(bad == nullptr, "conv2d_split: %s (nt %d, tile %d x %d)", bad ? bad : "", tile[0], tile[1], tile[2]);
+        nt = tile[0];
+        conv_set_tile(p, tile[1], tile[2], round_up(tile[2] + 3, 4));
+    } else {
+        const ConvPlan pl = conv_plan(p.P, p.Q, n, cout, rows_pad, true, conv_device_cus());
+        nt = pl.nt;
+        conv_set_tile(p, pl.th, pl.tw, pl.pwl);
+    }
     p.Opad = rows_pad;
     p.nkc_real = cdiv(cin, conv_bk(dtype, 3));
     p.nkc = terms * p.nkc_real;
@@ -2908,18 +3050,33 @@
     const bool small = (rows_pad % 128 != 0) || cout <= 64;
     const long long blocks = (long long)p.tilesX * p.tilesY * p.N * cdiv(p.Cout, small ? 64 : 128);
     AFCM_REQUIRE(blocks > 0 && blocks < (1ll << 31), "conv2d_split: grid of %lld blocks is out of range", blocks);
-    const dim3 block(256);
     hipStream_t st = (hipStream_t)stream;
     p.total_blocks = (int)blocks; p.o_base = 0;
     const dim3 pgrid(small ? (unsigned)conv_persistent_grid(blocks, 3) : (unsigned)blocks);
     if (dtype == AFCM_BF16) {
-        if (small) hipLaunchKernelGGL((conv2d_fwd16x_kernel<bf16_t, 64, true>), pgrid, block, 0, st, p);
-        else hipLaunchKernelGGL((conv2d_fwd16x_kernel<bf16_t, 128, true>), pgrid, block, 0, st, p);
+        if (small) launch_fwd16x<bf16_t, 64, true>(p, nt, pgrid, st);
+        else launch_fwd16x<bf16_t, 128, true>(p, nt, pgrid, st);
     } else {
-        if (small) hipLaunchKernelGGL((conv2d_fwd16x_kernel<f16_t, 64, true>), pgrid, block, 0, st, p);
-        else hipLaunchKernelGGL((conv2d_fwd16x_kernel<f16_t, 128, true>), pgrid, block, 0, st, p);
+        if (small) launch_fwd16x<f16_t, 64, true>(p, nt, pgrid, st);
+        else launch_fwd16x<f16_t, 128, true>(p, nt, pgrid, st);
     }
     return hip_status(hipGetLastError());
+}
+
+extern "C" int afcm_conv2d_split(float* y, const void* x_parts, const void* wpacked, const float* oscale, const float* obias, int32_t dtype, int32_t n,
+                                 int32_t cin, int32_t cout, int32_t h, int32_t w, int32_t pad, int32_t rows_pad, int32_t terms, uint32_t term_parts,
+                                 int64_t part_stride, const uint32_t* bound_a, const uint32_t* bound_b, void* stream) {
+    return conv2d_split_impl(y, x_parts, wpacked, oscale, obias, dtype, n, cin, cout, h, w, pad, rows_pad, terms, term_parts, part_stride, bound_a,
+                             bound_b, nullptr, stream);
+}
+
+extern "C" int afcm_conv2d_split_tile(float* y, const void* x_parts, const void* wpacked, const float* oscale, const float* obias, int32_t dtype,
+                                      int32_t n, int32_t cin, int32_t cout, int32_t h, int32_t w, int32_t pad, int32_t rows_pad, int32_t terms,
+                                      uint32_t term_parts, int64_t part_stride, const uint32_t* bound_a, const uint32_t* bound_b, int32_t nt,
+                                      int32_t th, int32_t tw, void* stream) {
+    const int tile[3] = {nt, th, tw};
+    return conv2d_split_impl(y, x_parts, wpacked, oscale, obias, dtype, n, cin, cout, h, w, pad, rows_pad, terms, term_parts, part_stride, bound_a,
+                             bound_b, tile, stream);
 }
 
 static int wgrad_rows_per_step(int dtype) { return dtype == AFCM_F32 ? 1 : 2; }
diff --git a/include/afcm_hip.h b/include/afcm_hip.h
--- a/include/afcm_hip.h
+++ b/include/afcm_hip.h
@@ -82,6 +82,11 @@
 int afcm_conv2d_ld(void* y, const void* x, const void* wpacked, const float* oscale, const float* obias, int32_t dtype, int32_t n,
                    int32_t cin, int32_t cout, int32_t h, int32_t w, int32_t ks, int32_t pad, int32_t rows_pad, int32_t x_pitch,
                    int32_t y_pitch, void* stream);
+int afcm_conv2d_plan(int32_t dtype, int32_t n, int32_t cin, int32_t cout, int32_t h, int32_t w, int32_t pad, int32_t rows_pad, int32_t split,
+                     int32_t cus, int32_t* plan, float* cost);
+int afcm_conv2d_tile_ld(void* y, const void* x, const void* wpacked, const float* oscale, const float* obias, int32_t dtype, int32_t n,
+                        int32_t cin, int32_t cout, int32_t h, int32_t w, int32_t pad, int32_t rows_pad, int32_t x_pitch, int32_t y_pitch,
+                        int32_t nt, int32_t th, int32_t tw, void* stream);
 
 int afcm_conv2d_wgrad_splits(int32_t n, int32_t cout, int32_t cin, int32_t p_rows);
 int afcm_conv2d_wgrad(float* dw, float* workspace, const void* dy, const void* x, int32_t dtype, int32_t n, int32_t cin,
@@ -190,6 +195,10 @@
 int afcm_conv2d_split(float* y, const void* x_parts, const void* wpacked, const float* oscale, const float* obias, int32_t dtype, int32_t n,
                       int32_t cin, int32_t cout, int32_t h, int32_t w, int32_t pad, int32_t rows_pad, int32_t terms, uint32_t term_parts,
                       int64_t part_stride, const uint32_t* bound_a, const uint32_t* bound_b, void* stream);
+int afcm_conv2d_split_tile(float* y, const void* x_parts, const void* wpacked, const float* oscale, const float* obias, int32_t dtype,
+                           int32_t n, int32_t cin, int32_t cout, int32_t h, int32_t w, int32_t pad, int32_t rows_pad, int32_t terms,
+                           uint32_t term_parts, int64_t part_stride, const uint32_t* bound_a, const uint32_t* bound_b, int32_t nt, int32_t th,
+                           int32_t tw, void* stream);
 
 int afcm_conv2d_stride2(void* y, const void* x, const void* wpacked, int32_t dtype, int32_t n, int32_t cin, int32_t cout, int32_t h, int32_t w,
                         int32_t pad, int32_t rows_pad, void* stream);
```

Result: no change. 487.1 images/sec (median of 6 runs) (+0.1%).
